# sahngmin/AdaptSegNet

Measured on AMD Instinct MI355X. Metric: adversarial-train images/sec at 1024×512, DeeplabMulti+D, 1/2/4/8 MI355X, higher is better.
Workload: dtype f32; 1 GPU; c2: DeeplabMulti single-level Vanilla, batch/GPU 4, source 1024x512, target 1024x512; global_batch=4, parallelism=dp1, conv_math=f32x3, x3h_mode=3, g16_wide=1, overlap_domains=True, overlap_d=False, target_first=False, d_reuse=True

## Files before the change

adaptsegnet_amd/_lib.py:

```python
from __future__ import annotations

import ctypes
import os
import re
import threading

_HERE = os.path.dirname(os.path.abspath(__file__))
LIB_PATH = os.environ.get("ADAPTSEG_LIBRARY") or os.path.join(_HERE, "lib", "libadaptseg.so")
HEADER_PATH = os.path.join(os.path.dirname(_HERE), "include", "adaptseg.h")

ADAPTSEG_OK = 0
EPI_LEAKY = 1
EPI_ACCUMULATE = 2
EPI_LEAKY_GRAD = 4
EPI_RESIDUAL = 8
EPI_RELU = 16
EPI_RELU_GRAD = 32
CONV_FWD, CONV_BWD_DATA, CONV_BWD_WEIGHT = 0, 1, 2
MATH_F32, MATH_BF16, MATH_BF16_WIDE, MATH_F32X3, MATH_F32X3_PRESPLIT = 0, 1, 2, 3, 4


class AdaptSegLibraryError(RuntimeError):
    pass


class ConvDesc(ctypes.Structure):
    _fields_ = [
        ("n", ctypes.c_int), ("c", ctypes.c_int), ("h", ctypes.c_int), ("w", ctypes.c_int),
        ("in_stride", ctypes.c_int64 * 4),
        ("k", ctypes.c_int), ("oh", ctypes.c_int), ("ow", ctypes.c_int),
        ("kh", ctypes.c_int), ("kw", ctypes.c_int),
        ("stride", ctypes.c_int), ("nseg", ctypes.c_int),
        ("pad", ctypes.c_int * 4), ("dil", ctypes.c_int * 4),
    ]


class OperandBN(ctypes.Structure):
    _fields_ = [("mean", ctypes.c_void_p), ("invstd", ctypes.c_void_p),
                ("weight", ctypes.c_void_p), ("bias", ctypes.c_void_p)]


class BnSumDesc(ctypes.Structure):
    _fields_ = [
        ("x", ctypes.c_void_p), ("x_bf16", ctypes.c_void_p),
        ("mean", ctypes.c_void_p), ("invstd", ctypes.c_void_p),
        ("weight", ctypes.c_void_p), ("bias", ctypes.c_void_p),
        ("bits", ctypes.c_void_p), ("mask", ctypes.c_int),
        ("partial", ctypes.c_void_p), ("partial_bytes", ctypes.c_size_t),
    ]


FUSE_MAX_MAPS = 8
FUSE_PROB, FUSE_LOGIT = 0, 1


class FuseDesc(ctypes.Structure):
    _fields_ = [
        ("n", ctypes.c_int), ("c", ctypes.c_int), ("oh", ctypes.c_int), ("ow", ctypes.c_int),
        ("nmaps", ctypes.c_int), ("mode", ctypes.c_int),
        ("h", ctypes.c_int * FUSE_MAX_MAPS), ("w", ctypes.c_int * FUSE_MAX_MAPS),
        ("mirror", ctypes.c_int * FUSE_MAX_MAPS),
        ("x", ctypes.c_void_p * FUSE_MAX_MAPS),
    ]


_P = ctypes.c_void_p
_I = ctypes.c_int
_L = ctypes.c_int64
_F = ctypes.c_float
_SZ = ctypes.c_size_t
_PP = ctypes.POINTER(ctypes.c_void_p)
_DESC = ctypes.POINTER(ConvDesc)

_SIGS = {
    "adaptseg_last_error": [],
    "adaptseg_version": [],
    "adaptseg_conv2d_workspace_size": [_DESC, _I, ctypes.POINTER(_SZ)],
    "adaptseg_conv2d_kernel_id": [_DESC, _I, ctypes.POINTER(_I), ctypes.POINTER(_I)],
    "adaptseg_conv2d_kernel_id_x": [_DESC, _I, _I, ctypes.POINTER(_I), ctypes.POINTER(_I)],
    "adaptseg_conv2d_copy_operand_only": [_DESC, _I, ctypes.POINTER(_I)],
    "adaptseg_conv2d_operand_bn_ok": [_DESC, _I, ctypes.POINTER(_I)],
    "adaptseg_conv2d_fwd_bnstats_abn": [_DESC, _P, ctypes.POINTER(OperandBN), _PP, _P, _P, _P, _SZ,
                                        ctypes.POINTER(ctypes.c_int), _P, _SZ, _P],
    "adaptseg_conv2d_bwd_weight_abn": [_DESC, _P, _P, ctypes.POINTER(OperandBN), _PP, _I, _P, _SZ, _P],
    "adaptseg_bn_fwd_train_tiles_stats": [_L, _I, _P, _I, _P, _P, _F, _F, _P, _P, _P],
    "adaptseg_conv2d_fwd": [_DESC, _P, _PP, _PP, _P, _P, _I, _P, _SZ, _P],
    "adaptseg_conv2d_bwd_data": [_DESC, _P, _PP, _P, _P, _P, _I, _P, _SZ, _P],
    "adaptseg_conv2d_bwd_weight": [_DESC, _P, _P, _PP, _PP, _I, _P, _SZ, _P],
    "adaptseg_conv2d_wpack_size": [_DESC, _I, ctypes.POINTER(_SZ)],
    "adaptseg_conv2d_wpack": [_DESC, _I, _PP, _P, _SZ, _P],
    "adaptseg_conv2d_fwd_x": [_DESC, _P, _P, _PP, _P, _PP, _P, _P, _P, _I, _P, _SZ, _P],
    "adaptseg_conv2d_fwd_bnstats_x": [_DESC, _P, _P, _PP, _P, _P, _P, _P, _SZ, ctypes.POINTER(ctypes.c_int), _P,
                                      _SZ, _P],
    "adaptseg_conv2d_bwd_data_x": [_DESC, _P, _P, _PP, _P, _P, _P, _P, _P, _I, _P, _SZ, _P],
    "adaptseg_conv2d_bwd_data_xg": [_DESC, _P, _P, _PP, _P, _P, _P, _P, _P, _P, _P, _I, _P, _SZ, _P],
    "adaptseg_conv2d_bwd_weight_x": [_DESC, _P, _P, _P, _P, _PP, _PP, _I, _P, _SZ, _P],
    "adaptseg_conv2d_bnsum_tiles": [_DESC, _I, ctypes.POINTER(_I)],
    "adaptseg_timing_reserve": [_L],
    "adaptseg_conv2d_bwd_data_bnsum": [_DESC, _P, _P, _PP, _P, _P, _P, _P, _P, _P, _I, ctypes.POINTER(BnSumDesc),
                                       ctypes.POINTER(_I), _P, _SZ, _P],
    "adaptseg_bn_bwd_sums": [_L, _I, _P, _P, _P, _P, _P, _P, _P, _P, _P, _P, _P, _P, _P, _P, _P, _I, _P, _I, _P, _SZ,
                             _P],
    "adaptseg_bn_fwd_train_x": [_L, _I, _P, _P, _P, _P, _P, _P, _F, _F, _P, _P, _P, _P, _P, _P, _I, _P, _SZ, _P],
    "adaptseg_bn_fwd_train_tiles_x": [_L, _I, _P, _I, _P, _P, _P, _P, _P, _P, _F, _F, _P, _P, _P, _P, _P, _P, _I,
                                      _P],
    "adaptseg_bn_fwd_infer_x": [_L, _I, _P, _P, _P, _P, _P, _P, _F, _P, _P, _P, _P, _I, _P],
    "adaptseg_bn_fwd_train_xm": [_L, _I, _P, _P, _P, _P, _P, _P, _F, _F, _P, _P, _P, _P, _P, _P, _P, _I, _P, _SZ,
                                 _P],
    "adaptseg_bn_fwd_train_tiles_xm": [_L, _I, _P, _I, _P, _P, _P, _P, _P, _P, _F, _F, _P, _P, _P, _P, _P, _P, _P,
                                       _I, _P],
    "adaptseg_bn_fwd_infer_xm": [_L, _I, _P, _P, _P, _P, _P, _P, _F, _P, _P, _P, _P, _P, _I, _P],
    "adaptseg_bn_bwd_x": [_L, _I, _P, _P, _P, _P, _P, _P, _P, _P, _P, _P, _P, _P, _I, _I, _P, _SZ, _P],
    "adaptseg_bn_bwd_xg": [_L, _I, _P, _P, _P, _P, _P, _P, _P, _P, _P, _P, _P, _P, _P, _P, _P, _I, _I, _P, _SZ, _P],
    "adaptseg_bn_workspace_size": [_L, _I, ctypes.POINTER(_SZ)],
    "adaptseg_bn_fwd_train": [_L, _I, _P, _P, _P, _P, _P, _F, _F, _P, _P, _P, _P, _I, _P, _SZ, _P],
    "adaptseg_upsample_argmax": [_I, _I, _I, _I, _I, _I, _P, _P, _P],
    "adaptseg_fuse_argmax": [ctypes.POINTER(FuseDesc), _P, _P, _P],
    "adaptseg_confusion_hist": [_L, _P, _P, _P, _I, _P, _P],
    "adaptseg_conf_hist": [_L, _P, _P, _I, _I, _P, _P],
    "adaptseg_pseudo_thresholds": [_P, _I, _I, ctypes.c_double, _F, _P, _P],
    "adaptseg_pseudo_label": [_L, _P, _P, _P, _I, _I, _P, _P, _P],
    "adaptseg_bn_fwd_train_tiles": [_L, _I, _P, _I, _P, _P, _P, _P, _P, _F, _F, _P, _P, _P, _P, _I, _P],
    "adaptseg_conv2d_bnstats_size": [_DESC, ctypes.POINTER(ctypes.c_size_t)],
    "adaptseg_conv2d_bnstats_tiles": [_DESC, ctypes.POINTER(_I)],
    "adaptseg_conv2d_bnstats_tiles_x": [_DESC, _I, ctypes.POINTER(_I)],
    "adaptseg_conv2d_fwd_bnstats": [_DESC, _P, _PP, _P, _P, _SZ, ctypes.POINTER(ctypes.c_int), _P, _SZ, _P],
    "adaptseg_bn_fwd_infer": [_L, _I, _P, _P, _P, _P, _P, _F, _P, _P, _I, _P],
    "adaptseg_bn_bwd": [_L, _I, _P, _P, _P, _P, _P, _P, _P, _P, _P, _I, _I, _P, _SZ, _P],
    "adaptseg_maxpool2d_fwd": [_I, _I, _I, _I, _I, _I, _I, _I, _I, _P, _P, _P, _P],
    "adaptseg_maxpool2d_bwd": [_I, _I, _I, _I, _I, _I, _I, _I, _I, _P, _P, _P, _P],
    "adaptseg_maxpool2d_fwd_x": [_I, _I, _I, _I, _I, _I, _I, _I, _I, _P, _P, _P, _P, _P],
    "adaptseg_maxpool2d_bwd_x": [_I, _I, _I, _I, _I, _I, _I, _I, _I, _P, _P, _P, _P, _P],
    "adaptseg_upsample_workspace_size": [_I, _I, _I, _I, _I, _I, ctypes.POINTER(_SZ)],
    "adaptseg_upsample_bilinear_fwd": [_I, _I, _I, _I, _I, _I, _P, _P, _P],
    "adaptseg_upsample_bilinear_bwd": [_I, _I, _I, _I, _I, _I, _P, _P, _I, _P, _SZ, _P],
    "adaptseg_softmax_fwd": [_L, _I, _P, _P, _P],
    "adaptseg_softmax_bwd": [_L, _I, _P, _P, _P, _I, _P],
    "adaptseg_ce_workspace_size": [_L, ctypes.POINTER(_SZ)],
    "adaptseg_softmax_ce_fwd": [_L, _I, _P, _P, _I, _P, _P, _P, _SZ, _P],
    "adaptseg_softmax_ce_bwd": [_L, _I, _P, _P, _I, _P, _P, _P, _P, _I, _P],
    "adaptseg_adv_workspace_size": [_L, ctypes.POINTER(_SZ)],
    "adaptseg_adv_loss_fwd": [_L, _P, _F, _I, _P, _P, _SZ, _P],
    "adaptseg_adv_loss_bwd": [_L, _P, _F, _I, _P, _P, _I, _P],
    "adaptseg_sgd_step": [_L, _P, _P, _P, _F, _F, _F, _F, _I, _I, _P],
    "adaptseg_adam_step": [_L, _P, _P, _P, _P, _F, _F, _F, _F, _I, _F, _P],
    "adaptseg_zero": [_P, _SZ, _P],
    "adaptseg_to_nhwc": [_I, _I, _I, _I, ctypes.POINTER(_L), _P, _P, _P],
    "adaptseg_to_nhwc_pad": [_I, _I, _I, _I, ctypes.POINTER(_L), _P, _I, _P, _I, _P],
    "adaptseg_axpy": [_L, _F, _P, _P, _I, _P],
    "adaptseg_add_i64": [_P, _L, _L, _P],
    "adaptseg_preprocess_workspace_size": [_I, _I, _I, _I, _I, ctypes.POINTER(_SZ)],
    "adaptseg_gta5_preprocess": [_I, _I, _I, _I, _I, _P, _F, _F, _F, _P, _P, _P, _P, _P, _SZ, _P],
    "adaptseg_preprocess_augment_workspace_size": [_I, _I, _I, _I, _I, ctypes.POINTER(ctypes.c_int32),
                                                   ctypes.POINTER(_SZ)],
    "adaptseg_gta5_preprocess_augment": [_I, _I, _I, _I, _I, _P, _F, _F, _F, _P, _P, _P, _P,
                                         ctypes.POINTER(ctypes.c_int32), _I, _P, _SZ, _P],
    "adaptseg_bn_bwd_affine": [_L, _I, _P, _P, _P, _P, _P, _P, _P, _P, _P, _I, _P, _P, _P, _SZ, _P],
    "adaptseg_up2_relu_cat_fwd": [_I, _I, _I, _I, _I, _P, _P, _P, _P],
    "adaptseg_up2_relu_cat_bwd": [_I, _I, _I, _I, _I, _P, _P, _P, _P, _P, _P],
    "adaptseg_grid_warp_fwd": [_I, _I, _I, _I, _I, _P, _P, _P, _P, _P, _P],
    "adaptseg_grid_warp_bwd_workspace_size": [_I, _I, _I, _I, ctypes.POINTER(_SZ)],
    "adaptseg_grid_warp_bwd": [_I, _I, _I, _I, _I, _P, _P, _P, _P, _P, _P, _P, _P, _P, _SZ, _P],
    "adaptseg_conv_set_math": [_I],
    "adaptseg_conv_get_math": [ctypes.POINTER(_I)],
    "adaptseg_conv_set_option": [_I, _I],
    "adaptseg_conv_get_option": [_I, ctypes.POINTER(_I)],
    "adaptseg_splitk_flush": [_P],
    "adaptseg_splitk_pending": [_P, ctypes.POINTER(_I)],
    "adaptseg_stream_create_cu_mask": [_I, _I, ctypes.POINTER(_P)],
    "adaptseg_stream_destroy": [_P],
    "adaptseg_timing_enable": [_I, _I],
    "adaptseg_timing_enable_mem": [_I],
    "adaptseg_timing_read_id": [_I, ctypes.POINTER(ctypes.c_double), ctypes.POINTER(ctypes.c_double),
                                ctypes.POINTER(_L)],
    "adaptseg_timing_read": [ctypes.POINTER(ctypes.c_double), ctypes.POINTER(ctypes.c_double),
                             ctypes.POINTER(_L)],
    "adaptseg_timing_enable_stream": [_I],
    "adaptseg_timing_read_id_stream": [_I, ctypes.POINTER(ctypes.c_double), ctypes.POINTER(_L)],
}
_RESTYPES = {"adaptseg_last_error": ctypes.c_char_p, "adaptseg_version": ctypes.c_char_p}

_lib = None
_lock = threading.Lock()


def header_symbols(path: str = HEADER_PATH) -> list[str]:
    text = open(path).read()
    text = re.sub(r"/\*.*?\*/", "", text, flags=re.S)
    return sorted(set(re.findall(r"\b(adaptseg_[a-z0-9_]+)\s*\(", text)))


def lib():
    global _lib
    if _lib is not None:
        return _lib
    with _lock:
        if _lib is not None:
            return _lib
        if not os.path.exists(LIB_PATH):
            raise AdaptSegLibraryError(
                f"{LIB_PATH} not found: build it with `make -C adaptsegnet_amd/csrc` "
                "(the HIP path has no CPU fallback)")
        try:
            L = ctypes.CDLL(LIB_PATH)
        except OSError as e:
            raise AdaptSegLibraryError(f"failed to load {LIB_PATH}: {e}") from e
        for name, argtypes in _SIGS.items():
            fn = getattr(L, name)
            fn.argtypes = argtypes
            fn.restype = _RESTYPES.get(name, ctypes.c_int)
        _lib = L
        return L


def check(status: int, what: str) -> None:
    if status != ADAPTSEG_OK:
        msg = lib().adaptseg_last_error().decode(errors="replace")
        raise RuntimeError(f"{what} failed (status {status}): {msg}")


def ptr_array(ptrs) -> "ctypes.Array":
    arr = (ctypes.c_void_p * 4)()
    for i, p in enumerate(ptrs):
        arr[i] = p
    return arr
```

adaptsegnet_amd/csrc/conv_igemm.hip:

```cpp
#include <atomic>
#include "conv_kernels.hpp"
#include "conv_thin.hpp"
#include <cstdlib>
#include <mutex>
#include <unordered_map>
#include <vector>

namespace adaptseg {

__global__ void splitk_reduce_kernel(const ConvParams p, const float *slab, int mode) {
  const size_t total = (size_t)p.M * p.N;
  for (size_t idx = blockIdx.x * (size_t)blockDim.x + threadIdx.x; idx < total;
       idx += (size_t)gridDim.x * blockDim.x) {
    float v = 0.f;
    for (int s = 0; s < p.splits; ++s) v += slab[(size_t)s * total + idx];
    int row = (int)(idx / p.N);
    int col = (int)(idx - (size_t)row * p.N);
    if (mode == MODE_WGRAD) {
      int seg = (int)fdiv((uint32_t)col, p.fd_nseg_k);
      int cc = col - seg * p.kseg;
      float *dst = seg == 0 ? p.dw[0] : seg == 1 ? p.dw[1] : seg == 2 ? p.dw[2] : p.dw[3];
      float *o = dst + (size_t)row * p.kseg + cc;
      *o = (p.flags & ADAPTSEG_EPI_ACCUMULATE) ? *o + v : v;
    } else {
// ... 775 lines not shown
static bool terms_in_epilogue(const Plan &pl, const uint16_t *yb, int64_t n) {
  return yb && is_x3(pl.family) && pl.p.N % 4 == 0 && 3 * n < (1ll << 31) && !(reinterpret_cast<uintptr_t>(yb) & 7);
}

static int out_copy(const float *y, uint16_t *yb, int64_t n, int C, hipStream_t s) {
  if (!yb || n == 0) return ADAPTSEG_OK;
  AS_CHECK_ARG(y, "conv: an operand copy needs the fp32 output on this path");
  const unsigned blocks = (unsigned)std::min<int64_t>(ceil_div(n, 256), 8192);
  if (copies_are_terms() && C % 4 == 0 && n / 4 < (1ll << 31) / 3 && aligned16(y) &&
      !(reinterpret_cast<uintptr_t>(yb) & 7))
    x3_out_copy4_kernel<<<(unsigned)std::min<int64_t>(ceil_div(n / 4, 256), 16384), 256, 0, s>>>(
        reinterpret_cast<const float4 *>(y), reinterpret_cast<uint2 *>(yb), (uint32_t)(n / 4), C / 4,
        make_fastdiv(C / 4));
  else if (copies_are_terms())
    x3_out_copy_kernel<<<blocks, 256, 0, s>>>(y, reinterpret_cast<__bf16 *>(yb), n, C);
  else
    bf16_out_copy_kernel<<<blocks, 256, 0, s>>>(y, reinterpret_cast<__bf16 *>(yb), n);
  AS_CHECK_LAUNCH("out_copy");
  return ADAPTSEG_OK;
}

bool use_thin(const adaptseg_conv_desc *d, int op) { return thin_eligible(d, op); }

static bool copy_only(const Plan &pl, const adaptseg_conv_desc *d, int op) {
  if (use_thin(d, op)) return false;
  if (tapgemm_eligible(d)) return tapgemm_copy_only(d, op);
  if (is_x3(pl.family)) return pl.terms_ok;
  return pl.family == Family::Bf16Dma || (pl.family == Family::Bf16 && op == ADAPTSEG_CONV_FWD);
}

static size_t plan_wpack_bytes(const Plan &pl) {
  if (pl.mode == MODE_WGRAD) return 0;
  if (is_x3(pl.family)) return x3_wpack_bytes(pl);
  if (is_bf16(pl.family)) return bf16_wpack_bytes(pl);
  return 0;
}

static int attach_wpack(Plan &pl, const void *w_pack) {
  pl.wpack_ext = nullptr;
  if (!w_pack || plan_wpack_bytes(pl) == 0) return ADAPTSEG_OK;
  AS_CHECK_ARG((reinterpret_cast<uintptr_t>(w_pack) & 15) == 0, "conv: weight pack must be 16-byte aligned");
  pl.wpack_ext = w_pack;
  return ADAPTSEG_OK;
}

static void finish_plan(Plan &pl, bool a_aligned, bool b_aligned, const void *act, const void *act2 = nullptr) {
  const bool two = pl.mode == MODE_WGRAD;
  const bool have = act && aligned16(act) && (!two || (act2 && aligned16(act2)));
  finish_plan(pl, Operands{a_aligned, b_aligned, have});
  pl.act_ext = have ? act : nullptr;
  pl.act_ext2 = have && two ? act2 : nullptr;
}

static int query_plan(const adaptseg_conv_desc *d, int op, const Operands &ops, Plan &pl) {
  const int st = make_plan(d, op, pl);
  if (st == ADAPTSEG_OK) finish_plan(pl, ops);
  return st;
}

}

using namespace adaptseg;

extern "C" {

int adaptseg_conv2d_workspace_size(const adaptseg_conv_desc *d, int op, size_t *bytes) {
  AS_CHECK_ARG(bytes, "null bytes");
  Plan base, pl;
  int st = make_plan(d, op, base);
  if (st) return st;
  size_t b = 0;
  for (const Operands &ops : {Operands{}, Operands{false, false, false}, Operands{true, true, true}}) {
    pl = base;
    finish_plan(pl, ops);
    b = std::max(b, pl.slab_bytes);
  }
  if (tapgemm_eligible(d)) b = std::max(b, tapgemm_workspace(d, op));
  if (use_thin(d, op)) b = std::max(b, thin_workspace(d, op));
  if (op == ADAPTSEG_CONV_BWD_WEIGHT) {
    int per, splits;
    bias_grad_split(d->n * d->oh * d->ow, d->k, &per, &splits);
    b = std::max(b, (size_t)splits * d->k * sizeof(float));
  }
  *bytes = b;
  return ADAPTSEG_OK;
}

int adaptseg_conv2d_kernel_id(const adaptseg_conv_desc *d, int op, int *kernel_id, int *splits) {
  AS_CHECK_ARG(kernel_id && splits, "conv2d_kernel_id: null");
  return adaptseg_conv2d_kernel_id_x(d, op, 0, kernel_id, splits);
}

int adaptseg_conv2d_kernel_id_x(const adaptseg_conv_desc *d, int op, int with_copies, int *kernel_id, int *splits) {
  AS_CHECK_ARG(kernel_id && splits, "conv2d_kernel_id_x: null");
  Plan pl;
  int st = query_plan(d, op, Operands{true, true, with_copies != 0}, pl);
  if (st) return st;
  if (use_thin(d, op)) {
    *kernel_id = thin_kernel_id(op);
    *splits = 1;
    return ADAPTSEG_OK;
  }
  if (tapgemm_eligible(d)) return tapgemm_kernel_id(d, op, kernel_id, splits);
  *kernel_id = ::adaptseg::kernel_id(pl, op);
  *splits = pl.p.splits;
  return ADAPTSEG_OK;
}

static bool abn_plan_ok(const Plan &pl, const adaptseg_conv_desc *d, int op) {
  if (d->c > kAbnMaxC || d->c % 4 || d->nseg != 1 || use_thin(d, op) || tapgemm_eligible(d)) return false;
  return (op == ADAPTSEG_CONV_FWD && pl.family == Family::X3Rows) ||
         (op == ADAPTSEG_CONV_BWD_WEIGHT && pl.family == Family::X3);
}

int adaptseg_conv2d_operand_bn_ok(const adaptseg_conv_desc *d, int op, int *ok) {
  AS_CHECK_ARG(ok, "conv2d_operand_bn_ok: null");
  *ok = 0;
  Plan pl;
  int st = query_plan(d, op, Operands{}, pl);
  if (st) return st;
  if (op != ADAPTSEG_CONV_FWD && op != ADAPTSEG_CONV_BWD_WEIGHT) return ADAPTSEG_OK;
  *ok = abn_plan_ok(pl, d, op) ? 1 : 0;
  return ADAPTSEG_OK;
}

static void set_abn(ConvParams &p, const adaptseg_operand_bn *abn) {
  p.abn_m = abn->mean;
  p.abn_is = abn->invstd;
  p.abn_w = abn->weight;
  p.abn_b = abn->bias;
}

int adaptseg_conv2d_copy_operand_only(const adaptseg_conv_desc *d, int op, int *only) {
  AS_CHECK_ARG(only, "conv2d_copy_operand_only: null");
  *only = 0;
  Plan pl;
  int st = make_plan(d, op, pl);
  if (st) return st;
  *only = copy_only(pl, d, op) ? 1 : 0;
  return ADAPTSEG_OK;
}

int adaptseg_conv2d_wpack_size(const adaptseg_conv_desc *d, int op, size_t *bytes) {
  AS_CHECK_ARG(bytes, "conv2d_wpack_size: null");
  *bytes = 0;
  Plan pl;
  int st = make_plan(d, op, pl);
  if (st) return st;
  if (use_thin(d, op) || tapgemm_eligible(d)) return ADAPTSEG_OK;
  *bytes = plan_wpack_bytes(pl);
  return ADAPTSEG_OK;
}

int adaptseg_conv2d_wpack(const adaptseg_conv_desc *d, int op, const float *const *w, void *pack, size_t bytes,
                          adaptseg_stream_t stream) {
  Plan pl;
  int st = make_plan(d, op, pl);
  if (st) return st;
  AS_CHECK_ARG(w && pack, "conv2d_wpack: null pointer");
  AS_CHECK_ARG((reinterpret_cast<uintptr_t>(pack) & 15) == 0, "conv2d_wpack: pack must be 16-byte aligned");
  const size_t need = (use_thin(d, op) || tapgemm_eligible(d)) ? 0 : plan_wpack_bytes(pl);
  AS_CHECK_ARG(need > 0, "conv2d_wpack: this product reads no weight pack (size 0)");
  AS_CHECK_ARG(bytes >= need, "conv2d_wpack: %zu bytes < %zu", bytes, need);
  for (int s = 0; s < d->nseg; ++s) {
    AS_CHECK_ARG(w[s], "conv2d_wpack: null weight %d", s);
    AS_CHECK_ARG(aligned16(w[s]), "conv2d_wpack: weight %d must be 16-byte aligned", s);
    pl.p.wt[s] = w[s];
  }
  const hipError_t e = is_x3(pl.family) ? prep_x3_wpack(pl, pack, as_stream(stream)) : prep_bf16_wpack(pl, pack, as_stream(stream));
  if (e != hipSuccess) {
    set_error("conv2d_wpack: %s", hipGetErrorString(e));
    return ADAPTSEG_ERR_HIP;
  }
  return ADAPTSEG_OK;
}

int adaptseg_conv2d_fwd(const adaptseg_conv_desc *d, const float *x, const float *const *w,
                        const float *const *bias, const float *res, float *y, int flags, void *ws,
                        size_t ws_bytes, adaptseg_stream_t stream) {
  return adaptseg_conv2d_fwd_x(d, x, nullptr, w, nullptr, bias, res, y, nullptr, flags, ws, ws_bytes, stream);
}

struct FwdStats {
  float *stats;
  size_t stats_bytes;
  int *ntiles;
  const adaptseg_operand_bn *abn;
};

static int fwd_impl(const adaptseg_conv_desc *d, const float *x, const uint16_t *x_bf16, const float *const *w,
                    const void *w_pack, const float *const *bias, const float *res, float *y, uint16_t *y_bf16,
                    int flags, void *ws, size_t ws_bytes, adaptseg_stream_t stream, const FwdStats *bn) {
  const char *who = bn ? "conv fwd_bnstats" : "conv fwd";
  if (bn) {
    AS_CHECK_ARG(bn->ntiles && bn->stats, "conv fwd_bnstats: null stats / ntiles");
    *bn->ntiles = 0;
  }
  Plan pl;
  int st = make_plan(d, ADAPTSEG_CONV_FWD, pl);
  if (st) return st;
  const bool thin = !bn && use_thin(d, ADAPTSEG_CONV_FWD);
  AS_CHECK_ARG((x || x_bf16) && w && (y || y_bf16), "%s: null pointer", who);
  AS_CHECK_ARG(y || !(thin || tapgemm_eligible(d)), "%s: this product needs the fp32 output%s", who,
               bn ? "" : " (thin / tap-GEMM path)");
  AS_CHECK_ARG(y || !(flags & ADAPTSEG_EPI_ACCUMULATE), "conv fwd: ACCUMULATE needs the fp32 output");
  AS_CHECK_ARG(x || copy_only(pl, d, ADAPTSEG_CONV_FWD),
               "%s: this product needs the fp32 input (no bf16-operand kernel for it)", who);
  AS_CHECK_ARG(!(flags & kEpiActGrad), "conv fwd: *_GRAD flags not valid");
  AS_CHECK_ARG(!((flags & ADAPTSEG_EPI_LEAKY) && (flags & ADAPTSEG_EPI_RELU)), "conv fwd: LEAKY and RELU");
  AS_CHECK_ARG(!(flags & ADAPTSEG_EPI_RESIDUAL) || res, "conv fwd: residual flag without res");
  for (int s = 0; s < d->nseg; ++s) AS_CHECK_ARG(w[s], "%s: null weight %d", who, s);
  AS_CHECK_ARG(!bn || !bn->abn || !tapgemm_eligible(d), "conv fwd_bnstats_abn: no operand-BN kernel for this product");
  if (bn && tapgemm_eligible(d))
    return fwd_impl(d, x, x_bf16, w, nullptr, nullptr, nullptr, y, y_bf16, 0, ws, ws_bytes, stream, nullptr);
  const int64_t ny = (int64_t)d->n * d->oh * d->ow * d->k;
  if (thin && thin_fwd(d, x, w[0], bias ? bias[0] : nullptr, res, y, flags, as_stream(stream)) == ADAPTSEG_OK)
    return out_copy(y, y_bf16, ny, d->k, as_stream(stream));
  if (tapgemm_eligible(d) && aligned16(x) && segs_aligned(w, d->nseg)) {
    st = tapgemm_fwd(d, x, x_bf16, w, bias, res, y, flags, ws, ws_bytes, as_stream(stream));
    return st ? st : out_copy(y, y_bf16, ny, d->k, as_stream(stream));
  }
  ConvParams &p = pl.p;
  p.x = x;
  for (int s = 0; s < d->nseg; ++s) {
    p.wt[s] = w[s];
    p.bias[s] = bias ? bias[s] : nullptr;
  }
  finish_plan(pl, aligned16(x), segs_aligned(w, d->nseg), x_bf16);
  AS_CHECK_ARG(x || (copy_only(pl, d, ADAPTSEG_CONV_FWD) && pl.act_ext),
               "%s: x is NULL but the plan (after the alignment checks) needs the fp32 input", who);
  if (bn && bn->abn) {
    AS_CHECK_ARG(abn_plan_ok(pl, d, ADAPTSEG_CONV_FWD),
                 "conv fwd_bnstats_abn: no operand-BN kernel for this product (adaptseg_conv2d_operand_bn_ok)");
    set_abn(p, bn->abn);
  }
  const bool terms = copies_are_terms();
  AS_CHECK_ARG(y || !terms, "%s: under the F32X3 maths the output is fp32%s", who,
               bn ? "" : " (y_bf16 is its term images)");
  const bool fused = terms && terms_in_epilogue(pl, y_bf16, ny);
  p.out = y;
  p.outb = (terms && !fused) ? nullptr : reinterpret_cast<__bf16 *>(y_bf16);
  p.outb_terms = fused ? 1 : 0;
  p.res = res;
  p.flags = flags;
  if (bn && pl.family != Family::Generic && p.splits == 1) {
    const int nt = (int)ceil_div(p.M, pl.tile.bm);
    if ((size_t)(nt + 2 * (int64_t)p.N * nt) * sizeof(float) <= bn->stats_bytes) {
      p.stats = bn->stats;
      p.stats_ntiles = nt;
      *bn->ntiles = nt;
    }
  }
  st = attach_wpack(pl, w_pack);
  if (st) return st;
  st = run_plan(pl, MODE_FWD, ws, ws_bytes, as_stream(stream));
  return (st || !terms || fused) ? st : out_copy(y, y_bf16, ny, d->k, as_stream(stream));
}

int adaptseg_conv2d_fwd_x(const adaptseg_conv_desc *d, const float *x, const uint16_t *x_bf16,
                          const float *const *w, const void *w_pack, const float *const *bias, const float *res,
                          float *y, uint16_t *y_bf16, int flags, void *ws, size_t ws_bytes,
                          adaptseg_stream_t stream) {
  return fwd_impl(d, x, x_bf16, w, w_pack, bias, res, y, y_bf16, flags, ws, ws_bytes, stream, nullptr);
}

int adaptseg_conv2d_bnstats_size(const adaptseg_conv_desc *d, size_t *bytes) {
  AS_CHECK_ARG(bytes, "conv2d_bnstats_size: null");
  int st = validate(d);
  if (st) return st;
  const int64_t m = (int64_t)d->n * d->oh * d->ow;
  const int64_t nt = ceil_div(m, 128);
  *bytes = (size_t)(nt + 2 * (int64_t)d->k * nt) * sizeof(float);
  return ADAPTSEG_OK;
}

int adaptseg_conv2d_bnstats_tiles(const adaptseg_conv_desc *d, int *ntiles) {
  return adaptseg_conv2d_bnstats_tiles_x(d, 0, ntiles);
}

int adaptseg_conv2d_bnstats_tiles_x(const adaptseg_conv_desc *d, int with_copy, int *ntiles) {
  AS_CHECK_ARG(ntiles, "conv2d_bnstats_tiles: null");
  *ntiles = 0;
  Plan pl;
  int st = query_plan(d, ADAPTSEG_CONV_FWD, Operands{true, true, with_copy != 0}, pl);
  if (st) return st;
  if (tapgemm_eligible(d)) return ADAPTSEG_OK;
  if (pl.family != Family::Generic && pl.p.splits == 1) *ntiles = (int)ceil_div(pl.p.M, pl.tile.bm);
  return ADAPTSEG_OK;
}

int adaptseg_conv2d_fwd_bnstats(const adaptseg_conv_desc *d, const float *x, const float *const *w, float *y,
                                float *stats, size_t stats_bytes, int *ntiles, void *ws, size_t ws_bytes,
                                adaptseg_stream_t stream) {
  return adaptseg_conv2d_fwd_bnstats_x(d, x, nullptr, w, nullptr, y, nullptr, stats, stats_bytes, ntiles, ws, ws_bytes,
                                       stream);
}

int adaptseg_conv2d_fwd_bnstats_x(const adaptseg_conv_desc *d, const float *x, const uint16_t *x_bf16,
                                  const float *const *w, const void *w_pack, float *y, uint16_t *y_bf16,
                                  float *stats, size_t stats_bytes, int *ntiles, void *ws, size_t ws_bytes,
                                  adaptseg_stream_t stream) {
  const FwdStats bn{stats, stats_bytes, ntiles, nullptr};
  return fwd_impl(d, x, x_bf16, w, w_pack, nullptr, nullptr, y, y_bf16, 0, ws, ws_bytes, stream, &bn);
}

int adaptseg_conv2d_fwd_bnstats_abn(const adaptseg_conv_desc *d, const float *x_pre, const adaptseg_operand_bn *abn,
                                    const float *const *w, const void *w_pack, float *y, float *stats,
                                    size_t stats_bytes, int *ntiles, void *ws, size_t ws_bytes,
                                    adaptseg_stream_t stream) {
  AS_CHECK_ARG(abn && abn->mean && abn->invstd && x_pre, "conv fwd_bnstats_abn: null operand BN / input");
  const FwdStats bn{stats, stats_bytes, ntiles, abn};
  return fwd_impl(d, x_pre, nullptr, w, w_pack, nullptr, nullptr, y, nullptr, 0, ws, ws_bytes, stream, &bn);
}

int adaptseg_conv2d_bwd_data(const adaptseg_conv_desc *d, const float *dy, const float *const *w,
                             const float *res, const float *aux, float *dx, int flags, void *ws,
                             size_t ws_bytes, adaptseg_stream_t stream) {
  return adaptseg_conv2d_bwd_data_x(d, dy, nullptr, w, nullptr, res, aux, dx, nullptr, flags, ws, ws_bytes, stream);
}

int adaptseg_conv2d_bwd_data_x(const adaptseg_conv_desc *d, const float *dy, const uint16_t *dy_bf16,
                               const float *const *w, const void *w_pack, const float *res, const float *aux,
                               float *dx, uint16_t *dx_bf16, int flags, void *ws, size_t ws_bytes,
                               adaptseg_stream_t stream) {
// ... 410 lines not shown
```

adaptsegnet_amd/csrc/conv_kernels.hpp:

```cpp
#pragma once
#include "common.hpp"
#include <algorithm>
#include <cstring>

namespace adaptseg {


typedef float floatx16 __attribute__((ext_vector_type(16)));

enum { MODE_FWD = 0, MODE_DGRAD = 1, MODE_WGRAD = 2 };
constexpr int kMaxTaps = 64;
constexpr int BK = 16;
constexpr int kX3BK = 16;
constexpr int kX3rBK = 32;
constexpr int x3_bn(int mode) { return 128; }
constexpr int x3_threads(int mode) { return 512; }

struct ConvParams {
  int M, N, K;
  int n, c, h, w;
  int sxn, sxc, sxh, sxw;
  int k, oh, ow;
  int stride;
  int ntaps, taps_per_seg, nseg;
  int kseg;
  int ktiles_per_split, splits;
  FastDiv fd_c, fd_k, fd_ow, fd_oh, fd_ohw, fd_hw, fd_w, fd_nseg_k;
  const float *x;
  const float *dy;
  const float *wt[4];
  float *out;
  float *dw[4];
  const float *bias[4];
  const float *res;
  const __bf16 *resb;
  const uint32_t *resbits;
  const float *aux;
  int flags;
  int kw_, kh_;
  int pad_[4], dil_[4];
  FastDiv fd_taps, fd_kw;
  __bf16 *outb;
  int outb_terms;
  float *stats;
  int stats_ntiles;
  float *bs_part;
  const float *bs_x;
  const __bf16 *bs_xb;
  const float *bs_mean, *bs_is, *bs_w, *bs_b;
  const uint32_t *bs_bits;
  int bs_mask, bs_ntiles;
  short tap_dy[kMaxTaps], tap_dx[kMaxTaps];
  const float *abn_m, *abn_is, *abn_w, *abn_b;
};
constexpr int kAbnMaxC = 512;

__device__ __forceinline__ float epi_prev(const ConvParams &p, size_t idx) {
  return p.out ? p.out[idx] : (float)p.outb[idx];
}
__device__ __forceinline__ void epi_outb(const ConvParams &p, size_t row, int col, float v) {
  if (p.outb_terms) {
    uint32_t h, m, l;
    split3_2(v, 0.f, h, m, l);
    __bf16 *o = p.outb + row * 3 * p.N + col;
    o[0] = __builtin_bit_cast(__bf16, (uint16_t)h);
    o[p.N] = __builtin_bit_cast(__bf16, (uint16_t)m);
    o[2 * p.N] = __builtin_bit_cast(__bf16, (uint16_t)l);
  } else {
    p.outb[row * p.N + col] = (__bf16)v;
  }
}
__device__ __forceinline__ float epi_res(const ConvParams &p, size_t idx) {
  const float r = p.resb ? (float)p.resb[idx] : p.res[idx];
  return (!p.resbits || ((p.resbits[idx >> 5] >> (idx & 31)) & 1u)) ? r : 0.f;
}


__device__ __forceinline__ float4 ld4(const float *p) { return *reinterpret_cast<const float4 *>(p); }

struct RowInfo {
  int base;
  int y0, x0;
  bool ok;
};

__device__ __forceinline__ RowInfo fwd_row_info(const ConvParams &p, int m) {
  RowInfo r;
  r.ok = m < p.M;
  int mm = r.ok ? m : 0;
  uint32_t t = fdiv((uint32_t)mm, p.fd_ow);
  int ow = mm - (int)t * p.ow;
  uint32_t b = fdiv(t, p.fd_oh);
  int oh = (int)t - (int)b * p.oh;
  r.base = (int)b * p.sxn;
  r.y0 = oh * p.stride;
  r.x0 = ow * p.stride;
  return r;
}

__device__ __forceinline__ float fwd_a_elem(const ConvParams &p, const short *tdy, const short *tdx,
                                            const RowInfo &r, int k) {
  if (!r.ok || k >= p.K) return 0.f;
  int tap = (int)fdiv((uint32_t)k, p.fd_c);
  int ci = k - tap * p.c;
  int ih = r.y0 + tdy[tap], iw = r.x0 + tdx[tap];
  if ((unsigned)ih >= (unsigned)p.h || (unsigned)iw >= (unsigned)p.w) return 0.f;
  return p.x[r.base + ih * p.sxh + iw * p.sxw + ci * p.sxc];
}

template <bool VEC>
__device__ __forceinline__ float4 fwd_a_load(const ConvParams &p, const short *tdy, const short *tdx,
                                             const RowInfo &r, int k) {
  if constexpr (VEC) {
    if (!r.ok || k >= p.K) return make_float4(0.f, 0.f, 0.f, 0.f);
    int tap = (int)fdiv((uint32_t)k, p.fd_c);
    int ci = k - tap * p.c;
    int ih = r.y0 + tdy[tap], iw = r.x0 + tdx[tap];
    if ((unsigned)ih >= (unsigned)p.h || (unsigned)iw >= (unsigned)p.w)
      return make_float4(0.f, 0.f, 0.f, 0.f);
    return ld4(p.x + r.base + ih * p.sxh + iw * p.sxw + ci);
  } else {
    return make_float4(fwd_a_elem(p, tdy, tdx, r, k), fwd_a_elem(p, tdy, tdx, r, k + 1),
                       fwd_a_elem(p, tdy, tdx, r, k + 2), fwd_a_elem(p, tdy, tdx, r, k + 3));
  }
}

__device__ __forceinline__ const float *seg_ptr(const ConvParams &p, int seg) {
  return seg == 0 ? p.wt[0] : seg == 1 ? p.wt[1] : seg == 2 ? p.wt[2] : p.wt[3];
}

__device__ __forceinline__ float fwd_b_elem(const ConvParams &p, int n, int k) {
  if (n >= p.N || k >= p.K) return 0.f;
  int seg = (int)fdiv((uint32_t)k, p.fd_nseg_k);
  int kk = k - seg * p.kseg;
  return seg_ptr(p, seg)[n * p.kseg + kk];
}

template <bool VEC>
__device__ __forceinline__ float4 fwd_b_load(const ConvParams &p, int n, int k) {
  if constexpr (VEC) {
    if (n >= p.N || k >= p.K) return make_float4(0.f, 0.f, 0.f, 0.f);
    int seg = (int)fdiv((uint32_t)k, p.fd_nseg_k);
    int kk = k - seg * p.kseg;
    return ld4(seg_ptr(p, seg) + n * p.kseg + kk);
  } else {
    return make_float4(fwd_b_elem(p, n, k), fwd_b_elem(p, n, k + 1), fwd_b_elem(p, n, k + 2),
                       fwd_b_elem(p, n, k + 3));
  }
}

__device__ __forceinline__ RowInfo dgrad_row_info(const ConvParams &p, int m) {
  RowInfo r;
  r.ok = m < p.M;
  int mm = r.ok ? m : 0;
  uint32_t t = fdiv((uint32_t)mm, p.fd_w);
  int iw = mm - (int)t * p.w;
  uint32_t b = fdiv(t, p.fd_hw);
  int ih = (int)t - (int)b * p.h;
  r.base = (int)b;
  r.y0 = ih;
  r.x0 = iw;
  return r;
}

__device__ __forceinline__ bool dgrad_src(const ConvParams &p, int v, int d, int lim, int &o) {
  int num = v - d;
  if (p.stride == 1) {
    o = num;
  } else {
    if (num < 0 || (num % p.stride) != 0) return false;
    o = num / p.stride;
  }
  return (unsigned)o < (unsigned)lim;
}

__device__ __forceinline__ float dgrad_a_elem(const ConvParams &p, const short *tdy, const short *tdx,
                                              const RowInfo &r, int k) {
  if (!r.ok || k >= p.K) return 0.f;
  int tap = (int)fdiv((uint32_t)k, p.fd_k);
  int co = k - tap * p.k;
  int oh, ow;
  if (!dgrad_src(p, r.y0, tdy[tap], p.oh, oh) || !dgrad_src(p, r.x0, tdx[tap], p.ow, ow)) return 0.f;
  return p.dy[((r.base * p.oh + oh) * p.ow + ow) * p.k + co];
}

template <bool VEC>
__device__ __forceinline__ float4 dgrad_a_load(const ConvParams &p, const short *tdy, const short *tdx,
                                               const RowInfo &r, int k) {
  if constexpr (VEC) {
    if (!r.ok || k >= p.K) return make_float4(0.f, 0.f, 0.f, 0.f);
    int tap = (int)fdiv((uint32_t)k, p.fd_k);
    int co = k - tap * p.k;
    int oh, ow;
    if (!dgrad_src(p, r.y0, tdy[tap], p.oh, oh) || !dgrad_src(p, r.x0, tdx[tap], p.ow, ow))
      return make_float4(0.f, 0.f, 0.f, 0.f);
    return ld4(p.dy + ((r.base * p.oh + oh) * p.ow + ow) * p.k + co);
  } else {
    return make_float4(dgrad_a_elem(p, tdy, tdx, r, k), dgrad_a_elem(p, tdy, tdx, r, k + 1),
                       dgrad_a_elem(p, tdy, tdx, r, k + 2), dgrad_a_elem(p, tdy, tdx, r, k + 3));
  }
}

__device__ __forceinline__ const float *dgrad_b_row(const ConvParams &p, int k) {
  int tap = (int)fdiv((uint32_t)k, p.fd_k);
  int co = k - tap * p.k;
  int seg = tap / p.taps_per_seg;
  int t = tap - seg * p.taps_per_seg;
  return seg_ptr(p, seg) + (co * p.taps_per_seg + t) * p.c;
}
// ... 1251 lines not shown
        d[2 * SA] = v.z;
        d[3 * SA] = v.w;
      } else {
        *reinterpret_cast<float4 *>(As + a_k[i] * SA + a_col[i]) = v;
      }
    }
#pragma unroll
    for (int i = 0; i < NQB; ++i) {
      const float4 v = mask4(mb[i], rb[i]);
      if constexpr (B_KC) {
        float *d = Bs + b_k[i] * SB + b_col[i];
        d[0] = v.x;
        d[SB] = v.y;
        d[2 * SB] = v.z;
        d[3 * SB] = v.w;
      } else {
        *reinterpret_cast<float4 *>(Bs + b_k[i] * SB + b_col[i]) = v;
      }
    }
  };

  const int lane = tid & 63, wave = tid >> 6;
  const int wm = wave / WAVES_N, wn = wave - wm * WAVES_N;
  const int l32 = lane & 31, hh = lane >> 5;

  floatx16 acc[TM][TN];
#pragma unroll
  for (int i = 0; i < TM; ++i)
#pragma unroll
    for (int j = 0; j < TN; ++j)
#pragma unroll
      for (int r = 0; r < 16; ++r) acc[i][j][r] = 0.f;

  if (kt0 < kt1) {
    load_tile(kt0);
    store_tile(0);
    __syncthreads();
    int cur = 0;
    for (int kt = kt0; kt < kt1; ++kt) {
      const bool more = kt + 1 < kt1;
      if (more) load_tile(kt + 1);
      const float *As = lds + cur * STAGE + wm * WTM + l32;
      const float *Bs = lds + cur * STAGE + BK * SA + wn * WTN + l32;
      float a[2][TM], b[2][TN];
#pragma unroll
      for (int i = 0; i < TM; ++i) a[0][i] = As[hh * SA + i * 32];
#pragma unroll
      for (int j = 0; j < TN; ++j) b[0][j] = Bs[hh * SB + j * 32];
      __builtin_amdgcn_s_setprio(1);
#pragma unroll
      for (int kk = 0; kk < BK; kk += 2) {
        const int cb = (kk >> 1) & 1;
        if (kk + 2 < BK) {
#pragma unroll
          for (int i = 0; i < TM; ++i) a[cb ^ 1][i] = As[(kk + 2 + hh) * SA + i * 32];
#pragma unroll
          for (int j = 0; j < TN; ++j) b[cb ^ 1][j] = Bs[(kk + 2 + hh) * SB + j * 32];
        }
        __builtin_amdgcn_sched_barrier(0);
#pragma unroll
        for (int i = 0; i < TM; ++i)
#pragma unroll
          for (int j = 0; j < TN; ++j)
            acc[i][j] = __builtin_amdgcn_mfma_f32_32x32x2f32(a[cb][i], b[cb][j], acc[i][j], 0, 0, 0);
      }
      __builtin_amdgcn_s_setprio(0);
      if (more) store_tile(cur ^ 1);
      __syncthreads();
      cur ^= 1;
    }
  }

  igemm_epilogue<MODE, BM, BN, WAVES_M, WAVES_N, S2>(p, acc, bm, bn, tm, tn, split, M, Hc, Wc, py, px, lds);
}


enum class Family {
  Generic,
  Fast,
  Bf16,
  Bf16Dma,
  X3,
  X3Terms,
  X3Rows,
};
inline bool is_x3(Family f) { return f == Family::X3 || f == Family::X3Terms || f == Family::X3Rows; }
inline bool is_bf16(Family f) { return f == Family::Bf16 || f == Family::Bf16Dma; }

struct Tile {
  int bm, bn, bk, threads;
};

struct Plan {
  ConvParams p;
  Family family;
  Tile tile;
  int cfg;
  bool va, vb;
  bool s2;
  bool ae, be;
  bool terms_ok;
  bool act_caller;
  const void *act_ext;
  const void *act_ext2;
  const void *wpack_ext;
  int mode;
  int tiles;
  size_t slab_bytes;
  double flops;
};

struct Operands {
  bool a_aligned = true, b_aligned = true;
  bool copies = false;
};

static const int kCfgBM[9] = {128, 256, 32, 64, 256, 64, 128, 256, 128};
static const int kCfgBN[9] = {128, 32, 256, 256, 64, 64, 128, 128, 128};
static const int kCfgThreads[9] = {256, 256, 256, 256, 256, 256, 256, 512, 256};
static int fast_bk(int cfg) { return (cfg == 4 || cfg == 6 || cfg == 8) ? 16 : 32; }


double conv_flops(const adaptseg_conv_desc *d);
int make_plan(const adaptseg_conv_desc *d, int op, Plan &pl);
void finish_plan(Plan &pl, const Operands &ops);
void set_splits(Plan &pl);
int kernel_id(const Plan &pl, int mode);
int run_plan(Plan &pl, int mode, void *ws, size_t ws_bytes, hipStream_t s, bool defer = false);

bool tapgemm_eligible(const adaptseg_conv_desc *d);
bool tapgemm_copy_only(const adaptseg_conv_desc *d, int op);
size_t tapgemm_workspace(const adaptseg_conv_desc *d, int op);
int tapgemm_kernel_id(const adaptseg_conv_desc *d, int op, int *kid, int *splits);
int tapgemm_fwd(const adaptseg_conv_desc *d, const float *x, const uint16_t *x_bf16, const float *const *w,
                const float *const *bias, const float *res, float *y, int flags, void *ws, size_t ws_bytes,
                hipStream_t s);
int tapgemm_bwd_data(const adaptseg_conv_desc *d, const float *dy, const float *const *w, const float *res,
                     const float *aux, float *dx, int flags, void *ws, size_t ws_bytes, hipStream_t s);
int tapgemm_bwd_weight(const adaptseg_conv_desc *d, const float *dy, const float *x, const uint16_t *x_bf16,
                       float *const *dw, int flags, void *ws, size_t ws_bytes, hipStream_t s);

hipError_t launch_fwd(const Plan &pl, hipStream_t s);
int conv_math();
size_t bf16_wpack_bytes(const Plan &pl);
size_t bf16_pre_bytes(const Plan &pl);
hipError_t prep_bf16(Plan &pl, void *ws, hipStream_t s);
hipError_t prep_bf16_wpack(const Plan &pl, void *pack, hipStream_t s);
hipError_t launch_bf16(const Plan &pl, void *ws, hipStream_t s);
size_t x3_wpack_bytes(const Plan &pl);
size_t x3_pre_bytes(const Plan &pl);
hipError_t prep_x3(const Plan &pl, void *wpack, hipStream_t s);
hipError_t prep_x3_wpack(const Plan &pl, void *pack, hipStream_t s);
hipError_t launch_x3(const Plan &pl, void *wpack, hipStream_t s);
hipError_t launch_dgrad(const Plan &pl, hipStream_t s);
hipError_t launch_wgrad(const Plan &pl, hipStream_t s);

}
```

adaptsegnet_amd/csrc/conv_launch_bf16.hip:

```cpp
#include "conv_bf16.hpp"
#include "conv_bf16g.hpp"

namespace adaptseg {

__global__ void conv_wpack_fwd_kernel(const ConvParams p, __bf16 *out) {
  const int ktot = p.nseg * p.kseg;
  const int64_t n = (int64_t)p.k * ktot;
  for (int64_t i = (int64_t)blockIdx.x * blockDim.x + threadIdx.x; i < n; i += (int64_t)gridDim.x * blockDim.x) {
    const int co = (int)(i / ktot), kk = (int)(i - (int64_t)co * ktot);
    const int seg = kk / p.kseg, tk = kk - seg * p.kseg;
    out[i] = (__bf16)seg_ptr(p, seg)[(size_t)co * p.kseg + tk];
  }
}

__global__ void __launch_bounds__(256) conv_wpack_dgrad_kernel(const ConvParams p, __bf16 *out) {
  __shared__ float tile[64][65];
  const int ci0 = blockIdx.x * 64, co0 = blockIdx.y * 64, tap = blockIdx.z;
  const int seg = tap / p.taps_per_seg, t = tap - seg * p.taps_per_seg;
  const float *w = seg_ptr(p, seg);
  const int tx = threadIdx.x & 63, ty = threadIdx.x >> 6;
  for (int r = ty; r < 64; r += 4) {
    const int co = co0 + r, ci = ci0 + tx;
    tile[r][tx] = (co < p.k && ci < p.c) ? w[((size_t)co * p.taps_per_seg + t) * p.c + ci] : 0.f;
  }
  __syncthreads();
  const size_t ktot = (size_t)p.ntaps * p.k;
  for (int r = ty; r < 64; r += 4) {
    const int ci = ci0 + r, co = co0 + tx;
    if (ci < p.c && co < p.k) out[(size_t)ci * ktot + (size_t)tap * p.k + co] = (__bf16)tile[tx][r];
  }
}

__global__ void __launch_bounds__(256) conv_wpack_fwd_v_kernel(const ConvParams p, uint4 *__restrict__ out,
                                                               uint32_t cpr, uint32_t total) {
  for (uint32_t i = blockIdx.x * 256u + threadIdx.x; i < total; i += gridDim.x * 256u) {
    const uint32_t co = i / cpr, k0 = (i - co * cpr) * 8;
    int seg = 0;
    uint32_t tk = k0;
    while (tk >= (uint32_t)p.kseg) { tk -= p.kseg; ++seg; }
    const float *src = seg_ptr(p, seg) + (size_t)co * p.kseg + tk;
    const uint2 lo = cvt4_bf16(ld4(src)), hi = cvt4_bf16(ld4(src + 4));
    out[i] = make_uint4(lo.x, lo.y, hi.x, hi.y);
  }
}

__global__ void __launch_bounds__(256) conv_wpack_dgrad_v_kernel(const ConvParams p, __bf16 *out) {
  __shared__ float tile[64][65];
  const int ci0 = blockIdx.x * 64, co0 = blockIdx.y * 64, tap = blockIdx.z;
  const int seg = tap / p.taps_per_seg, t = tap - seg * p.taps_per_seg;
  const float *w = seg_ptr(p, seg);
  const int f = threadIdx.x & 15, r0 = threadIdx.x >> 4;
#pragma unroll
  for (int j = 0; j < 4; ++j) {
    const int r = r0 + 16 * j, co = co0 + r, ci = ci0 + 4 * f;
    float4 v = make_float4(0.f, 0.f, 0.f, 0.f);
    if (co < p.k && ci < p.c) v = ld4(w + ((size_t)co * p.taps_per_seg + t) * p.c + ci);
    tile[r][4 * f] = v.x; tile[r][4 * f + 1] = v.y; tile[r][4 * f + 2] = v.z; tile[r][4 * f + 3] = v.w;
  }
  __syncthreads();
  const size_t ktot = (size_t)p.ntaps * p.k;
  const int c = threadIdx.x & 7, co = co0 + 8 * c;
#pragma unroll
  for (int j = 0; j < 2; ++j) {
    const int rl = (threadIdx.x >> 3) + 32 * j, ci = ci0 + rl;
    if (ci >= p.c || co >= p.k) continue;
    const float *col = &tile[8 * c][rl];
    const uint2 lo = cvt4_bf16(make_float4(col[0], col[65], col[130], col[195]));
    const uint2 hi = cvt4_bf16(make_float4(col[260], col[325], col[390], col[455]));
    *reinterpret_cast<uint4 *>(out + (size_t)ci * ktot + (size_t)tap * p.k + co) = make_uint4(lo.x, lo.y, hi.x, hi.y);
  }
}

__global__ void bf16_copy_kernel(const float *__restrict__ x, int n, int h, int w, int c8, int sxn, int sxh,
                                 int sxw, uint4 *__restrict__ out) {
  const int64_t total = (int64_t)n * h * w * c8;
  for (int64_t i = (int64_t)blockIdx.x * blockDim.x + threadIdx.x; i < total; i += (int64_t)gridDim.x * blockDim.x) {
    const int cq = (int)(i % c8);
    const int64_t pix = i / c8;
    const int xx = (int)(pix % w);
    const int64_t t = pix / w;
    const int yy = (int)(t % h), b = (int)(t / h);
    const float *src = x + (int64_t)b * sxn + (int64_t)yy * sxh + (int64_t)xx * sxw + 8 * cq;
    const uint2 lo = cvt4_bf16(ld4(src)), hi = cvt4_bf16(ld4(src + 4));
    out[i] = make_uint4(lo.x, lo.y, hi.x, hi.y);
  }
}

static size_t g16_act_elems(const Plan &pl) {
  const ConvParams &p = pl.p;
  if (pl.family != Family::Bf16Dma) return 0;
  return pl.mode == MODE_FWD ? (size_t)p.n * p.h * p.w * p.c : (size_t)p.n * p.oh * p.ow * p.k;
}
static size_t g16_act2_elems(const Plan &pl) {
  const ConvParams &p = pl.p;
  return pl.family == Family::Bf16Dma && pl.mode == MODE_WGRAD ? (size_t)p.n * p.h * p.w * p.c : 0;
}
static size_t al256(size_t b) { return (b + 255) / 256 * 256; }

size_t bf16_pre_bytes(const Plan &pl) {
  return al256(bf16_wpack_bytes(pl)) + al256(g16_act_elems(pl) * sizeof(__bf16)) +
         al256(g16_act2_elems(pl) * sizeof(__bf16));
}

size_t bf16_wpack_bytes(const Plan &pl) {
  const ConvParams &p = pl.p;
  if (pl.mode == MODE_FWD) return (size_t)p.k * p.nseg * p.kseg * sizeof(__bf16);
  if (pl.mode == MODE_DGRAD) return (size_t)p.c * p.ntaps * p.k * sizeof(__bf16);
  return 0;
}

hipError_t prep_bf16_wpack(const Plan &pl, void *pack, hipStream_t s) {
  const ConvParams &p = pl.p;
  __bf16 *wb = reinterpret_cast<__bf16 *>(pack);
  bool wal = true;
  for (int g = 0; g < p.nseg; ++g) wal = wal && (reinterpret_cast<uintptr_t>(p.wt[g]) & 15) == 0;
  if (pl.mode == MODE_FWD) {
    const int64_t n = (int64_t)p.k * p.nseg * p.kseg;
    if (wal && p.kseg % 8 == 0 && n / 8 < (int64_t)1 << 31) {
      const uint32_t total = (uint32_t)(n / 8);
      conv_wpack_fwd_v_kernel<<<(unsigned)std::min<int64_t>(ceil_div(total, 256), 4096), 256, 0, s>>>(
          p, reinterpret_cast<uint4 *>(wb), (uint32_t)(p.nseg * p.kseg / 8), total);
    } else {
      conv_wpack_fwd_kernel<<<(unsigned)std::min<int64_t>(ceil_div(n, 256), 4096), 256, 0, s>>>(p, wb);
    }
  } else if (pl.mode == MODE_DGRAD) {
    dim3 g((unsigned)ceil_div(p.c, 64), (unsigned)ceil_div(p.k, 64), (unsigned)p.ntaps);
    if (wal && p.c % 4 == 0 && p.k % 8 == 0) conv_wpack_dgrad_v_kernel<<<g, 256, 0, s>>>(p, wb);
    else conv_wpack_dgrad_kernel<<<g, 256, 0, s>>>(p, wb);
  }
  return hipGetLastError();
}

hipError_t prep_bf16(Plan &pl, void *wpack, hipStream_t s) {
  const ConvParams &p = pl.p;
  if (!pl.wpack_ext) {
    const hipError_t e = prep_bf16_wpack(pl, wpack, s);
    if (e != hipSuccess) return e;
  }
  if (pl.family == Family::Bf16Dma) {
    char *base = reinterpret_cast<char *>(wpack) + al256(bf16_wpack_bytes(pl));
    uint4 *act = reinterpret_cast<uint4 *>(base);
    const int64_t n8 = (int64_t)g16_act_elems(pl) / 8;
    const unsigned blocks = (unsigned)std::min<int64_t>(ceil_div(n8, 256), 8192);
    if (!pl.act_ext) {
      if (pl.mode == MODE_FWD)
        bf16_copy_kernel<<<blocks, 256, 0, s>>>(p.x, p.n, p.h, p.w, p.c / 8, p.sxn, p.sxh, p.sxw, act);
      else
        bf16_copy_kernel<<<blocks, 256, 0, s>>>(p.dy, p.n, p.oh, p.ow, p.k / 8, p.oh * p.ow * p.k, p.ow * p.k,
                                                p.k, act);
    }
    if (pl.mode == MODE_WGRAD && !pl.act_ext2) {
      uint4 *act2 = reinterpret_cast<uint4 *>(base + al256(g16_act_elems(pl) * sizeof(__bf16)));
      const int64_t m8 = (int64_t)g16_act2_elems(pl) / 8;
      bf16_copy_kernel<<<(unsigned)std::min<int64_t>(ceil_div(m8, 256), 8192), 256, 0, s>>>(
          p.x, p.n, p.h, p.w, p.c / 8, p.sxn, p.sxh, p.sxw, act2);
    }
  }
  return hipGetLastError();
}

hipError_t launch_bf16(const Plan &pl, void *wpack, hipStream_t s) {
  const ConvParams &p = pl.p;
  const __bf16 *wb = reinterpret_cast<const __bf16 *>(pl.wpack_ext ? pl.wpack_ext : wpack);
  const Tile &t = pl.tile;
  const bool bn256 = t.bn == 256;
  dim3 grid(pl.tiles, p.splits, pl.s2 ? 4 : 1), block(t.threads);
  if (pl.family == Family::Bf16Dma) {
    const char *base = reinterpret_cast<const char *>(wpack) + al256(bf16_wpack_bytes(pl));
    const __bf16 *act = reinterpret_cast<const __bf16 *>(pl.act_ext ? pl.act_ext : base);
    if (pl.s2) {
      if (bn256) launch_k(igemm_bf16g_kernel<MODE_DGRAD, 128, 256, 32, true>, grid, block, s, p, act, wb);
      else launch_k(igemm_bf16g_kernel<MODE_DGRAD, 256, 128, 32, true>, grid, block, s, p, act, wb);
    } else if (pl.mode == MODE_WGRAD) {
      const __bf16 *act2 = reinterpret_cast<const __bf16 *>(
          pl.act_ext2 ? pl.act_ext2 : base + al256(g16_act_elems(pl) * sizeof(__bf16)));
      if (bn256) launch_k(igemm_bf16g_wgrad_kernel<256, 256, 2>, grid, block, s, p, act, act2);
      else if (t.bm == 256) launch_k(igemm_bf16g_wgrad_kernel<256>, grid, block, s, p, act, act2);
      else launch_k(igemm_bf16g_wgrad_kernel<128>, grid, block, s, p, act, act2);
    } else {
#define G16_LAUNCH(MODE_, BK_)                                                                     \
  do {                                                                                             \
    if (t.bm == 256 && bn256)                                                                      \
      launch_k(igemm_bf16g_kernel<MODE_, 256, 256, 64, false, 2>, grid, block, s, p, act, wb);     \
    else if (bn256) launch_k(igemm_bf16g_kernel<MODE_, 128, 256, BK_>, grid, block, s, p, act, wb); \
    else launch_k(igemm_bf16g_kernel<MODE_, 256, 128, BK_>, grid, block, s, p, act, wb);           \
  } while (0)
      if (pl.mode == MODE_FWD && t.bk == 64) G16_LAUNCH(MODE_FWD, 64);
      else if (pl.mode == MODE_FWD) G16_LAUNCH(MODE_FWD, 32);
      else if (t.bk == 64) G16_LAUNCH(MODE_DGRAD, 64);
      else G16_LAUNCH(MODE_DGRAD, 32);
#undef G16_LAUNCH
    }
    return hipGetLastError();
  }
  const __bf16 *act = pl.mode == MODE_FWD ? reinterpret_cast<const __bf16 *>(pl.act_ext) : nullptr;
  if (pl.mode == MODE_FWD && act) {
    if (bn256) launch_k(igemm_bf16_kernel<MODE_FWD, false, 256, true>, grid, block, s, p, wb, act);
    else launch_k(igemm_bf16_kernel<MODE_FWD, false, 128, true>, grid, block, s, p, wb, act);
  } else if (pl.mode == MODE_FWD) {
    if (bn256) launch_k(igemm_bf16_kernel<MODE_FWD, false, 256>, grid, block, s, p, wb, act);
    else launch_k(igemm_bf16_kernel<MODE_FWD, false, 128>, grid, block, s, p, wb, act);
  } else if (pl.mode == MODE_DGRAD && pl.s2) {
    if (bn256) launch_k(igemm_bf16_kernel<MODE_DGRAD, true, 256>, grid, block, s, p, wb, act);
    else launch_k(igemm_bf16_kernel<MODE_DGRAD, true, 128>, grid, block, s, p, wb, act);
  } else if (pl.mode == MODE_DGRAD) {
    if (bn256) launch_k(igemm_bf16_kernel<MODE_DGRAD, false, 256>, grid, block, s, p, wb, act);
    else launch_k(igemm_bf16_kernel<MODE_DGRAD, false, 128>, grid, block, s, p, wb, act);
  } else {
    launch_k(igemm_bf16_kernel<MODE_WGRAD, false, 128>, grid, block, s, p, wb, act);
  }
  return hipGetLastError();
}

}
```

adaptsegnet_amd/csrc/conv_launch_x3.hip:

```cpp
#include "conv_x3r.hpp"

namespace adaptseg {

static void x3_pack_dims(const Plan &pl, int &rows_pad, int &ktot) {
  const ConvParams &p = pl.p;
  rows_pad = ktot = 0;
  if (pl.mode == MODE_FWD) {
    rows_pad = (int)ceil_div(p.k, x3_bn(MODE_FWD)) * x3_bn(MODE_FWD);
    ktot = p.nseg * p.kseg;
  } else if (pl.mode == MODE_DGRAD) {
    rows_pad = (int)ceil_div(p.c, x3_bn(MODE_DGRAD)) * x3_bn(MODE_DGRAD);
    ktot = p.ntaps * p.k;
  }
}

size_t x3_wpack_bytes(const Plan &pl) {
  int rows_pad, ktot;
  x3_pack_dims(pl, rows_pad, ktot);
  return 3 * (size_t)rows_pad * ktot * sizeof(__bf16);
}

static size_t x3_act_elems(const Plan &pl) {
  const ConvParams &p = pl.p;
  if (pl.family != Family::X3Terms) return 0;
  return pl.mode == MODE_FWD ? (size_t)p.n * p.h * p.w * p.c : (size_t)p.n * p.oh * p.ow * p.k;
}
static size_t x3_act2_elems(const Plan &pl) {
  const ConvParams &p = pl.p;
  return pl.family == Family::X3Terms && pl.mode == MODE_WGRAD ? (size_t)p.n * p.h * p.w * p.c : 0;
}
static size_t al256(size_t b) { return (b + 255) / 256 * 256; }

size_t x3_pre_bytes(const Plan &pl) {
  if (pl.act_caller) return al256(x3_wpack_bytes(pl));
  return al256(x3_wpack_bytes(pl)) + al256(3 * x3_act_elems(pl) * sizeof(__bf16)) +
         al256(3 * x3_act2_elems(pl) * sizeof(__bf16));
}

static void split_copy(const float *x, int n, int h, int w, int c, int sxn, int sxh, int sxw, void *out,
                       hipStream_t s) {
  const int64_t n8 = (int64_t)n * h * w * c / 8;
  x3_split_copy_kernel<<<(unsigned)std::min<int64_t>(ceil_div(n8, 256), 8192), 256, 0, s>>>(
      x, n, h, w, c / 8, sxn, sxh, sxw, reinterpret_cast<uint4 *>(out));
}

hipError_t prep_x3_wpack(const Plan &pl, void *pack, hipStream_t s) {
  const ConvParams &p = pl.p;
  int rows_pad, ktot;
  x3_pack_dims(pl, rows_pad, ktot);
  const dim3 pg((unsigned)(rows_pad / x3_bn(pl.mode)), (unsigned)(ktot / kX3BK));
  if (pl.mode == MODE_FWD) conv_wpack_x3v_kernel<MODE_FWD><<<pg, 256, 0, s>>>(p, (char *)pack, ktot);
  else if (pl.mode == MODE_DGRAD) conv_wpack_x3v_kernel<MODE_DGRAD><<<pg, 256, 0, s>>>(p, (char *)pack, ktot);
  return hipGetLastError();
}

hipError_t prep_x3(const Plan &pl, void *wpack, hipStream_t s) {
  const ConvParams &p = pl.p;
  if (!pl.wpack_ext) {
    const hipError_t e = prep_x3_wpack(pl, wpack, s);
    if (e != hipSuccess) return e;
  }
  if (pl.family == Family::X3Terms) {
    char *base = reinterpret_cast<char *>(wpack) + al256(x3_wpack_bytes(pl));
    if (!pl.act_ext) {
      if (pl.mode == MODE_FWD) split_copy(p.x, p.n, p.h, p.w, p.c, p.sxn, p.sxh, p.sxw, base, s);
      else split_copy(p.dy, p.n, p.oh, p.ow, p.k, p.oh * p.ow * p.k, p.ow * p.k, p.k, base, s);
    }
    if (pl.mode == MODE_WGRAD && !pl.act_ext2)
      split_copy(p.x, p.n, p.h, p.w, p.c, p.sxn, p.sxh, p.sxw, base + al256(3 * x3_act_elems(pl) * sizeof(__bf16)),
                 s);
  }
  return hipGetLastError();
}

hipError_t launch_x3(const Plan &pl, void *wpack, hipStream_t s) {
  const ConvParams &p = pl.p;
  const __bf16 *wb = reinterpret_cast<const __bf16 *>(pl.wpack_ext ? pl.wpack_ext : wpack);
  const int mode = pl.mode;
  dim3 grid(pl.tiles, p.splits, pl.s2 ? 4 : 1), block(pl.tile.threads);
  switch (pl.family) {
    case Family::X3Terms: {
      const char *base = reinterpret_cast<const char *>(wpack) + al256(x3_wpack_bytes(pl));
      const __bf16 *act = reinterpret_cast<const __bf16 *>(pl.act_ext ? pl.act_ext : base);
      if (mode == MODE_FWD) launch_k(igemm_x3r_kernel<MODE_FWD, false>, grid, block, s, p, act, wb);
      else if (mode == MODE_DGRAD && pl.s2) launch_k(igemm_x3r_kernel<MODE_DGRAD, true>, grid, block, s, p, act, wb);
      else if (mode == MODE_DGRAD) launch_k(igemm_x3r_kernel<MODE_DGRAD, false>, grid, block, s, p, act, wb);
      else {
        const __bf16 *act2 = reinterpret_cast<const __bf16 *>(
            pl.act_ext2 ? pl.act_ext2 : base + al256(3 * x3_act_elems(pl) * sizeof(__bf16)));
        if (pl.tile.bm == 256) launch_k(igemm_x3r_wgrad_kernel<256>, grid, block, s, p, act, act2);
        else launch_k(igemm_x3r_wgrad_kernel<128>, grid, block, s, p, act, act2);
      }
      break;
    }
    case Family::X3Rows:
      if (mode == MODE_WGRAD) launch_k(igemm_x3hw_kernel<128>, grid, block, s, p);
      else if (mode == MODE_FWD && p.abn_m) launch_k(igemm_x3h_abn_kernel, grid, block, s, p, wb);
      else if (mode == MODE_FWD) launch_k(igemm_x3h_kernel<MODE_FWD, false>, grid, block, s, p, wb);
      else if (pl.s2) launch_k(igemm_x3h_kernel<MODE_DGRAD, true>, grid, block, s, p, wb);
      else launch_k(igemm_x3h_kernel<MODE_DGRAD, false>, grid, block, s, p, wb);
      break;
    case Family::X3:
      if (mode == MODE_FWD) launch_k(igemm_x3_kernel<MODE_FWD, false>, grid, block, s, p, wb);
      else if (mode == MODE_DGRAD && pl.s2) launch_k(igemm_x3_kernel<MODE_DGRAD, true>, grid, block, s, p, wb);
      else if (mode == MODE_DGRAD) launch_k(igemm_x3_kernel<MODE_DGRAD, false>, grid, block, s, p, wb);
      else if (p.abn_m) launch_k(igemm_x3_abn_kernel, grid, block, s, p, wb);
      else launch_k(igemm_x3_kernel<MODE_WGRAD, false>, grid, block, s, p, wb);
      break;
    default: return hipErrorInvalidValue;
  }
  return hipGetLastError();
}

}
```

adaptsegnet_amd/csrc/conv_x3.hpp:

```cpp
#pragma once
#include "conv_bf16.hpp"


namespace adaptseg {

constexpr int kX3Img = 128 * kX3BK * 2;

__device__ __forceinline__ int kc16_off(int r, int ch) { return r * 32 + ((ch ^ ((r >> 3) & 1)) << 4); }

__device__ __forceinline__ bf16x8 kc16_frag(const char *img, int r0, int lane) {
  return as_bf16x8(*reinterpret_cast<const uint4 *>(img + kc16_off(r0 + (lane & 31), lane >> 5)));
}

typedef unsigned int u32x4 __attribute__((ext_vector_type(4)));
static __device__ __attribute__((aligned(16))) float g_x3_zero4[4];

template <int MODE, bool S2, bool ABN>
__device__ __forceinline__ void x3_body(const ConvParams &p, const __bf16 *__restrict__ wb) {
  static_assert(!ABN || MODE == MODE_WGRAD, "operand BN: the weight gradient's x operand");
  constexpr bool MC = MODE == MODE_WGRAD;
  constexpr int BM = 128, BN = 128, BK = kX3BK, NT = x3_threads(MODE);
  constexpr int WAVES_M = 2, WAVES_N = NT / 128;
  constexpr int WTM = BM / WAVES_M, WTN = BN / WAVES_N;
  constexpr int TM = WTM / 32, TN = WTN / 32;
// ... 204 lines not shown
        uint2 h, m, l;
        split3(ra[i], h, m, l);
        *reinterpret_cast<uint2 *>(As + o) = h;
        *reinterpret_cast<uint2 *>(As + IMG + o) = m;
        *reinterpret_cast<uint2 *>(As + 2 * IMG + o) = l;
        split3(rbf[i], h, m, l);
        *reinterpret_cast<uint2 *>(Bs + o) = h;
        *reinterpret_cast<uint2 *>(Bs + IMGB + o) = m;
        *reinterpret_cast<uint2 *>(Bs + 2 * IMGB + o) = l;
      }
    }
  };

  const int lane = tid & 63, wave = tid >> 6;
  const int wm = wave / WAVES_N, wn = wave - wm * WAVES_N;
  uint32_t mca[MC ? TM : 1][2], mcb[MC ? TN : 1][2];
  if constexpr (MC) {
    const int g = lane >> 4, i16 = lane & 15, q = i16 >> 2, pp = i16 & 3;
    const int kb = 8 * (g >> 1);
    auto offs = [&](int c0, uint32_t (&o)[2]) {
      const int ch = ((c0 + 16 * (g & 1)) >> 3) + (pp >> 1);
      o[0] = (uint32_t)(mc_off(kb + q, ch) + 8 * (pp & 1));
      o[1] = (uint32_t)(mc_off(kb + 4 + q, ch) + 8 * (pp & 1));
    };
#pragma unroll
    for (int i = 0; i < TM; ++i) offs(wm * WTM + i * 32, mca[i]);
#pragma unroll
    for (int j = 0; j < TN; ++j) offs(wn * WTN + j * 32, mcb[j]);
  }
  const uint32_t lds_u32 = (uint32_t)(uintptr_t)lds;
  auto mc_read = [&](uint32_t img_base, const uint32_t (&o)[2]) -> bf16x8 {
    const bf16x4 t0 = __builtin_amdgcn_ds_read_tr16_b64_v4bf16((lds_bf16x4 *)(uintptr_t)(img_base + o[0]));
    const bf16x4 t1 = __builtin_amdgcn_ds_read_tr16_b64_v4bf16((lds_bf16x4 *)(uintptr_t)(img_base + o[1]));
    return __builtin_shufflevector(t0, t1, 0, 1, 2, 3, 4, 5, 6, 7);
  };

  floatx16 acc[TM][TN];
#pragma unroll
  for (int i = 0; i < TM; ++i)
#pragma unroll
    for (int j = 0; j < TN; ++j)
#pragma unroll
      for (int r = 0; r < 16; ++r) acc[i][j][r] = 0.f;
  floatx16 accs[TM][TN];
#pragma unroll
  for (int i = 0; i < TM; ++i)
#pragma unroll
    for (int j = 0; j < TN; ++j)
#pragma unroll
      for (int r = 0; r < 16; ++r) accs[i][j][r] = 0.f;

  auto abn_x = [&]() {
    if constexpr (ABN) {
      const float *L = reinterpret_cast<const float *>(lds + 2 * STAGE) + b_off[0];
      const float4 bm4 = *reinterpret_cast<const float4 *>(L);
      const float4 bi4 = *reinterpret_cast<const float4 *>(L + kAbnMaxC);
      const float4 bw4 = *reinterpret_cast<const float4 *>(L + 2 * kAbnMaxC);
      const float4 bb4 = *reinterpret_cast<const float4 *>(L + 3 * kAbnMaxC);
      float4 &xv = rbf[0];
      xv.x = rbv ? bn_relu(xv.x, bm4.x, bi4.x, bw4.x, bb4.x) : 0.f;
      xv.y = rbv ? bn_relu(xv.y, bm4.y, bi4.y, bw4.y, bb4.y) : 0.f;
      xv.z = rbv ? bn_relu(xv.z, bm4.z, bi4.z, bw4.z, bb4.z) : 0.f;
      xv.w = rbv ? bn_relu(xv.w, bm4.w, bi4.w, bw4.w, bb4.w) : 0.f;
    }
  };
  auto compute = [&](auto cur_c) {
    constexpr int cur = decltype(cur_c)::value;
    const char *As = lds + cur * STAGE;
    const char *Bs = As + 3 * IMG;
    abn_x();
    bf16x8 a[3][TM], b[3][TN];
#pragma unroll
    for (int s = 0; s < 3; ++s) {
#pragma unroll
      for (int i = 0; i < TM; ++i) {
        if constexpr (MC) a[s][i] = mc_read(lds_u32 + cur * STAGE + s * IMG, mca[i]);
        else a[s][i] = kc16_frag(As + s * IMG, wm * WTM + i * 32, lane);
      }
#pragma unroll
      for (int j = 0; j < TN; ++j) {
        if constexpr (MC) b[s][j] = mc_read(lds_u32 + cur * STAGE + 3 * IMG + s * IMGB, mcb[j]);
        else b[s][j] = kc16_frag(Bs + s * IMGB, wn * WTN + j * 32, lane);
      }
    }
    constexpr int TA[6] = {0, 0, 1, 0, 1, 2};
    constexpr int TB[6] = {0, 1, 0, 2, 1, 0};
    __builtin_amdgcn_s_setprio(1);
#pragma unroll
    for (int u = 0; u < 6; ++u)
#pragma unroll
      for (int i = 0; i < TM; ++i)
#pragma unroll
        for (int j = 0; j < TN; ++j) {
          if (u == 0) acc[i][j] = __builtin_amdgcn_mfma_f32_32x32x16_bf16(a[0][i], b[0][j], acc[i][j], 0, 0, 0);
          else accs[i][j] = __builtin_amdgcn_mfma_f32_32x32x16_bf16(a[TA[u]][i], b[TB[u]][j], accs[i][j], 0, 0, 0);
        }
    store_tile(std::integral_constant<int, cur ^ 1>{});
#pragma unroll
    for (int q = 0; q < 6 * TM * TN; ++q) {
      __builtin_amdgcn_sched_group_barrier(0x008, 1, 0);
      __builtin_amdgcn_sched_group_barrier(0x002, 3, 0);
      __builtin_amdgcn_sched_group_barrier(0x200, 1, 0);
    }
    __builtin_amdgcn_s_setprio(0);
  };

  if constexpr (ABN) {
    float *L = reinterpret_cast<float *>(lds + 2 * STAGE);
    for (int c = tid; c < p.c; c += NT) {
      L[c] = p.abn_m[c];
      L[kAbnMaxC + c] = p.abn_is[c];
      L[2 * kAbnMaxC + c] = p.abn_w ? p.abn_w[c] : 1.f;
      L[3 * kAbnMaxC + c] = p.abn_b ? p.abn_b[c] : 0.f;
    }
    __syncthreads();
  }
  if (kt0 < kt1) {
    const int klast = kt1 - 1;
    load_tile(kt0);
    abn_x();
    store_tile(std::integral_constant<int, 0>{});
    load_tile(min(kt0 + 1, klast));
    __syncthreads();
    for (int kt = kt0; kt < kt1; kt += 2) {
      compute(std::integral_constant<int, 0>{});
      load_tile(min(kt + 2, klast));
      __syncthreads();
      if (kt + 1 >= kt1) break;
      compute(std::integral_constant<int, 1>{});
      load_tile(min(kt + 3, klast));
      __syncthreads();
    }
  }

#pragma unroll
  for (int i = 0; i < TM; ++i)
#pragma unroll
    for (int j = 0; j < TN; ++j) acc[i][j] += accs[i][j];
  static_assert(sizeof(lds) >= WAVES_M * WAVES_N * 32 * 36 * 4, "LDS for the f32x4 epilogue");
  igemm_epilogue<MODE, BM, BN, WAVES_M, WAVES_N, S2, 2>(p, acc, bm, bn, tm, tn, split, M, Hc, Wc, py, px,
                                                      reinterpret_cast<float *>(lds));
}

template <int MODE, bool S2>
__global__ void __launch_bounds__(x3_threads(MODE), 4) igemm_x3_kernel(const ConvParams p, const __bf16 *__restrict__ wb) {
  x3_body<MODE, S2, false>(p, wb);
}
__global__ void __launch_bounds__(x3_threads(MODE_WGRAD), 4) igemm_x3_abn_kernel(const ConvParams p,
                                                                               const __bf16 *__restrict__ wb) {
  x3_body<MODE_WGRAD, false, true>(p, wb);
}

template <int MODE>
__global__ void __launch_bounds__(256) conv_wpack_x3v_kernel(const ConvParams p, char *out, int ktot) {
  constexpr int TR = x3_bn(MODE), IMGB = TR * kX3BK * 2;
  const int r = threadIdx.x >> 1, ch = threadIdx.x & 1;
  const int n = blockIdx.x * TR + r;
  const int ks = blockIdx.y, k0 = ks * kX3BK + 8 * ch;
  float v[8];
  if constexpr (MODE == MODE_FWD) {
    if (n < p.k) {
      const int seg = k0 / p.kseg;
      const float *src = seg_ptr(p, seg) + (size_t)n * p.kseg + (k0 - seg * p.kseg);
      const float4 a = ld4(src), b = ld4(src + 4);
      v[0] = a.x; v[1] = a.y; v[2] = a.z; v[3] = a.w; v[4] = b.x; v[5] = b.y; v[6] = b.z; v[7] = b.w;
    } else {
#pragma unroll
      for (int j = 0; j < 8; ++j) v[j] = 0.f;
    }
  } else {
    const int tap = k0 / p.k, co = k0 - tap * p.k;
    const int seg = tap / p.taps_per_seg, t = tap - seg * p.taps_per_seg;
    const float *src = seg_ptr(p, seg) + ((size_t)co * p.taps_per_seg + t) * p.c + n;
    const size_t cs = (size_t)p.taps_per_seg * p.c;
#pragma unroll
    for (int j = 0; j < 8; ++j) v[j] = n < p.c ? src[j * cs] : 0.f;
  }
  uint4 h, m, l;
  split3_2(v[0], v[1], h.x, m.x, l.x);
  split3_2(v[2], v[3], h.y, m.y, l.y);
  split3_2(v[4], v[5], h.z, m.z, l.z);
  split3_2(v[6], v[7], h.w, m.w, l.w);
  const int nkt = ktot / kX3BK;
  char *dst = out + ((size_t)blockIdx.x * nkt + ks) * 3 * IMGB + kc16_off(r, ch);
  *reinterpret_cast<uint4 *>(dst) = h;
  *reinterpret_cast<uint4 *>(dst + IMGB) = m;
  *reinterpret_cast<uint4 *>(dst + 2 * IMGB) = l;
}

}
```

adaptsegnet_amd/kernels.py:

```python
from __future__ import annotations

import contextlib
import ctypes
import weakref
from dataclasses import dataclass

import torch

from . import _lib
from . import ops as _ops
from ._lib import (CONV_BWD_DATA, CONV_BWD_WEIGHT, CONV_FWD, EPI_ACCUMULATE, EPI_LEAKY,
                   EPI_LEAKY_GRAD, EPI_RELU, EPI_RELU_GRAD, EPI_RESIDUAL, MATH_BF16, MATH_BF16_WIDE, MATH_F32, MATH_F32X3, MATH_F32X3_PRESPLIT,
                   ConvDesc, check)

__all__ = [
    "ConvGeom", "set_conv_math", "get_conv_math", "MATH_F32", "MATH_BF16", "MATH_BF16_WIDE", "MATH_F32X3", "MATH_F32X3_PRESPLIT", "conv_fwd", "conv_fwd_bnstats", "conv_dgrad", "conv_wgrad", "bn_fwd_train",
    "bn_fwd_train_tiles", "bn_fwd_infer", "bn_bwd",
    "maxpool_fwd", "maxpool_bwd", "upsample_fwd", "upsample_bwd", "softmax_fwd", "softmax_bwd",
    "ce_fwd", "ce_bwd", "adv_fwd", "adv_bwd", "sgd_step", "adam_step", "zero_", "to_nhwc",
    "axpy", "add_i64", "weight_pack_scope", "pack_builds", "pack_count", "clear_weight_packs", "EPI_ACCUMULATE", "EPI_LEAKY", "EPI_LEAKY_GRAD", "EPI_RELU", "EPI_RELU_GRAD", "EPI_RESIDUAL",
]


_OP = _ops.OPS
_p, _stream, _ws_args, workspace = _ops._p, _ops._stream, _ops._ws_args, _ops.workspace


def _require(t: torch.Tensor, what: str):
    if not t.is_cuda:
        raise RuntimeError(f"{what}: expected a CUDA (HIP) tensor, got device {t.device}")
    if t.dtype != torch.float32:
        raise RuntimeError(f"{what}: expected float32, got {t.dtype}")


@dataclass(frozen=True)
class ConvGeom:

    cin: int
    cout: int
    kh: int
    kw: int
    stride: int = 1
    pads: tuple = (0,)
    dils: tuple = (1,)

    @property
    def nseg(self) -> int:
        return len(self.pads)

    def out_hw(self, h: int, w: int):
        p, d = self.pads[0], self.dils[0]
        oh = (h + 2 * p - d * (self.kh - 1) - 1) // self.stride + 1
        ow = (w + 2 * p - d * (self.kw - 1) - 1) // self.stride + 1
        return oh, ow

    def flops(self, n: int, h: int, w: int) -> float:
        oh, ow = self.out_hw(h, w)
        return 2.0 * n * oh * ow * self.cout * self.cin * self.kh * self.kw * self.nseg


def set_conv_math(math: int) -> None:
    _ops.set_math(math)


def set_x3h(mode: int) -> None:
    _ops.set_option(_ops.OPT_X3H, mode)


def get_x3h() -> int:
    return _ops.get_option(_ops.OPT_X3H)


def set_g16_wide(mode) -> None:
    _ops.set_option(_ops.OPT_G16_WIDE, 3 if mode is True else int(mode))


def get_g16_wide() -> int:
    return _ops.get_option(_ops.OPT_G16_WIDE)


def get_conv_math() -> int:
    m = ctypes.c_int(0)
    check(_lib.lib().adaptseg_conv_get_math(ctypes.byref(m)), "conv_get_math")
    return m.value


def _desc(g: ConvGeom, n, h, w, strides):
    return _ops.conv_desc(n, g.cin, h, w, strides, g.cout, g.kh, g.kw, g.stride, g.pads, g.dils)


class _PackCache:

    def __init__(self):
        self.depth = 0
        self.epoch = 0
        self.entries = {}
        self.finalizers = {}
        self.sizes = {}
        self.builds = 0

    def _drop(self, wid):
        self.entries.pop(wid, None)
        self.finalizers.pop(wid, None)

    def track(self, weight):
        wid = id(weight)
        per = self.entries.get(wid)
        if per is None:
            per = self.entries[wid] = {}
            f = self.finalizers.get(wid)
            if f is None or not f.alive:
                self.finalizers[wid] = weakref.finalize(weight, self._drop, wid)
        return per


_PACKS = _PackCache()


@contextlib.contextmanager
def weight_pack_scope():
    _PACKS.depth += 1
    try:
        yield
    finally:
        _PACKS.depth -= 1
        if _PACKS.depth == 0:
            _PACKS.epoch += 1


def pack_builds() -> int:
    return _PACKS.builds


def pack_count() -> int:
    return sum(len(v) for v in list(_PACKS.entries.values()))


def clear_weight_packs() -> None:
    _PACKS.entries.clear()


def _wpack(g, n, h, w, strides, weights, op):
    if _PACKS.depth == 0:
        return None
    if not _aligned16(*weights):
        return None
    math = _ops._CONV_MATH[0]
    skey = (g, op, math, strides[1] == 1)
    size = _PACKS.sizes.get(skey)
    if size is None:
        d = _desc(g, n, h, w, tuple(strides))[0]
        b = ctypes.c_size_t(0)
        check(_lib.lib().adaptseg_conv2d_wpack_size(ctypes.byref(d), op, ctypes.byref(b)), "conv2d_wpack_size")
        size = _PACKS.sizes[skey] = b.value
    if size == 0:
        return None
    per = _PACKS.track(weights[0])
    key = (tuple(t.data_ptr() for t in weights), g, op, math)
    e = per.get(key)
    if e is None or e[0].numel() < size:
        e = per[key] = [torch.empty(size, dtype=torch.uint8, device=weights[0].device), -1]
    if e[1] != _PACKS.epoch:
        _OP.conv2d_wpack(list(weights), e[0], (n, g.cin, h, w), tuple(strides), _wshape(g), g.stride, g.pads,
                         g.dils, op)
        e[1] = _PACKS.epoch
        _PACKS.builds += 1
    return e[0]


def nhwc_strides(n, h, w, c):
    return (h * w * c, 1, w * c, c)


def _wshape(g: ConvGeom):
    return (g.cout, g.cin, g.kh, g.kw)


def conv_fwd(g: ConvGeom, x: torch.Tensor, n: int, h: int, w: int, weights, biases=None,
             strides=None, out=None, res=None, flags: int = 0, xb=None, bf16_out: bool = False,
             bf16_only: bool = False):
    strides = strides or nhwc_strides(n, h, w, g.cin)
    oh, ow = g.out_hw(h, w)
    dev = (x if x is not None else xb).device
    if bf16_only:
        outb = torch.empty((n, oh, ow, g.cout), device=dev, dtype=torch.bfloat16)
        wp = _wpack(g, n, h, w, strides, weights, CONV_FWD)
        _OP.conv2d_fwd(x, xb, list(weights), wp, list(biases) if biases is not None else [], res, None, outb,
                       (n, g.cin, h, w), strides, _wshape(g), g.stride, g.pads, g.dils,
                       flags | (EPI_RESIDUAL if res is not None else 0))
        return outb
    if out is None:
        out = torch.empty((n, oh, ow, g.cout), device=dev, dtype=torch.float32)
    if res is not None:
        flags |= EPI_RESIDUAL
    outb = _bf16_like(out, bf16_out)
    wp = _wpack(g, n, h, w, strides, weights, CONV_FWD)
    _OP.conv2d_fwd(x, xb, list(weights), wp, list(biases) if biases is not None else [], res, out, outb,
                   (n, g.cin, h, w), strides, _wshape(g), g.stride, g.pads, g.dils, flags)
    return (out, outb) if bf16_out else out


def conv_bnstats_tiles(g: ConvGeom, n: int, h: int, w: int, strides, with_copy: bool = False) -> int:
    d = _desc(g, n, h, w, tuple(strides))[0]
    nt = ctypes.c_int(0)
    check(_lib.lib().adaptseg_conv2d_bnstats_tiles_x(ctypes.byref(d), 1 if with_copy else 0, ctypes.byref(nt)),
          "conv2d_bnstats_tiles")
    return nt.value


def conv_fwd_bnstats(g: ConvGeom, x: torch.Tensor, n: int, h: int, w: int, weights, strides=None, xb=None,
                     bf16_only: bool = False):
    strides = tuple(strides or nhwc_strides(n, h, w, g.cin))
    nt = conv_bnstats_tiles(g, n, h, w, strides, with_copy=xb is not None and _aligned16(xb))
    if nt == 0 or not _aligned16(x, *weights):
        return conv_fwd(g, x, n, h, w, weights, strides=strides, xb=xb, bf16_only=bf16_only), None
    oh, ow = g.out_hw(h, w)
    dev = (x if x is not None else xb).device
    shape = (n, oh, ow, g.cout)
    out = None if bf16_only else torch.empty(shape, device=dev, dtype=torch.float32)
    outb = torch.empty(shape, device=dev, dtype=torch.bfloat16) if bf16_only else None
    stats = torch.empty(nt * (1 + 2 * g.cout), device=dev, dtype=torch.float32)
    wp = _wpack(g, n, h, w, strides, weights, CONV_FWD)
    _OP.conv2d_fwd_bnstats(x, xb, list(weights), wp, out, outb, stats, (n, g.cin, h, w), strides, _wshape(g),
                           g.stride, g.pads, g.dils, nt)
    return (outb if bf16_only else out), (stats, nt)


def _aligned16(*ts) -> bool:
    return all(t is None or t.data_ptr() % 16 == 0 for t in ts)


@dataclass
class OperandBN:
    mean: torch.Tensor
    invstd: torch.Tensor
    weight: torch.Tensor | None
    bias: torch.Tensor | None


def operand_bn_ok(g: ConvGeom, n: int, h: int, w: int, op: int) -> bool:
    return _ops.operand_bn_ok((n, g.cin, h, w), nhwc_strides(n, h, w, g.cin), _wshape(g), g.stride, g.pads, g.dils,
                              op)


def conv_fwd_bnstats_abn(g: ConvGeom, x_pre: torch.Tensor, abn: OperandBN, n: int, h: int, w: int, weights):
    strides = nhwc_strides(n, h, w, g.cin)
    nt = conv_bnstats_tiles(g, n, h, w, strides)
    if nt == 0 or not _aligned16(x_pre, *weights):
        raise RuntimeError("conv_fwd_bnstats_abn: no fused-statistics plan for this product / unaligned operand")
    oh, ow = g.out_hw(h, w)
    out = torch.empty((n, oh, ow, g.cout), device=x_pre.device, dtype=torch.float32)
    stats = torch.empty(nt * (1 + 2 * g.cout), device=x_pre.device, dtype=torch.float32)
    wp = _wpack(g, n, h, w, strides, weights, CONV_FWD)
    _OP.conv2d_fwd_bnstats_abn(x_pre, abn.mean, abn.invstd, abn.weight, abn.bias, list(weights), wp, out, stats,
                               (n, g.cin, h, w), strides, _wshape(g), g.stride, g.pads, g.dils, nt)
    return out, (stats, nt)


def conv_wgrad_abn(g: ConvGeom, dy: torch.Tensor, x_pre: torch.Tensor, abn: OperandBN, n: int, h: int, w: int, dws,
                   accumulate: bool = True) -> None:
    _OP.conv2d_bwd_weight_abn(dy, x_pre, abn.mean, abn.invstd, abn.weight, abn.bias, list(dws), (n, g.cin, h, w),
                              nhwc_strides(n, h, w, g.cin), _wshape(g), g.stride, g.pads, g.dils,
                              EPI_ACCUMULATE if accumulate else 0)


def conv_bnsum_tiles(g: ConvGeom, n: int, h: int, w: int, with_copy: bool = False) -> int:
    d = _desc(g, n, h, w, nhwc_strides(n, h, w, g.cin))[0]
    nt = ctypes.c_int(0)
    check(_lib.lib().adaptseg_conv2d_bnsum_tiles(ctypes.byref(d), 1 if with_copy else 0, ctypes.byref(nt)),
          "conv2d_bnsum_tiles")
    return nt.value


@dataclass
class BnSum:
    x: torch.Tensor
    mean: torch.Tensor
    invstd: torch.Tensor
    weight: torch.Tensor | None
    bias: torch.Tensor | None
    mask: int
    bits: torch.Tensor | None = None


BNSUM_NONE, BNSUM_RELU_X, BNSUM_BITS = 0, 1, 2


def conv_dgrad(g: ConvGeom, dy: torch.Tensor, n: int, h: int, w: int, weights, out=None,
               res=None, aux=None, flags: int = 0, dyb=None, bf16_out: bool = False, bf16_only: bool = False,
               resbits=None, bnsum: BnSum | None = None):
    low = bf16_only or (out is not None and out.dtype == torch.bfloat16)
    dev = (dy if dy is not None else dyb).device
    if out is None:
        out = torch.empty((n, h, w, g.cin), device=dev, dtype=torch.bfloat16 if low else torch.float32)
    if res is not None:
        flags |= EPI_RESIDUAL
    if aux is not None and not flags & EPI_RELU_GRAD:
        assert not low, "conv_dgrad: aux with bf16 gradient storage is not a supported combination"
        flags |= EPI_LEAKY_GRAD
    outb = None if low else _bf16_like(out, bf16_out)
    dx, dxb = (None, out) if low else (out, outb)
    wp = _wpack(g, n, h, w, nhwc_strides(n, h, w, g.cin), weights, CONV_BWD_DATA)
    ret = out if (low or not bf16_out) else (out, outb)
    nt = 0
    if (bnsum is not None and aux is None and g.cin % 4 == 0 and _aligned16(dy, *weights) and
            _aligned16(bnsum.mean, bnsum.invstd, bnsum.weight, bnsum.bias) and
            (bnsum.x is None or bnsum.x.dtype != torch.float32 or _aligned16(bnsum.x))):
        nt = conv_bnsum_tiles(g, n, h, w, with_copy=dyb is not None and _aligned16(dyb))
    if nt == 0:
        _OP.conv2d_bwd_data(dy, dyb, list(weights), wp, res, resbits, aux, dx, dxb, (n, g.cin, h, w), _wshape(g),
                            g.stride, g.pads, g.dils, flags)
        return ret if bnsum is None else (ret, None)
    partial = torch.empty(2 * g.cin * nt, device=dev, dtype=torch.float32)
    b = bnsum
    _OP.conv2d_bwd_data_bnsum(dy, dyb, list(weights), wp, res, resbits, dx, dxb, (n, g.cin, h, w), _wshape(g),
                              g.stride, g.pads, g.dils, flags, b.x, b.mean, b.invstd, b.weight, b.bias, b.bits,
                              int(b.mask), partial, nt)
    return ret, (partial, nt)

# ... 336 lines not shown
```

adaptsegnet_amd/ops.py:

```python
from __future__ import annotations

import ctypes

import torch

from . import _lib
from ._lib import CONV_BWD_DATA, CONV_BWD_WEIGHT, CONV_FWD, MATH_F32X3, ConvDesc, check

LIB = torch.library.Library("adaptseg", "DEF")


def _stream() -> ctypes.c_void_p:
    return ctypes.c_void_p(torch.cuda.current_stream().cuda_stream)


def _p(t):
    return None if t is None else ctypes.c_void_p(t.data_ptr())


def _pf(t, n, what):
    if t is None:
        return None
    if t.dtype != torch.float32 or t.numel() != n:
        raise RuntimeError(f"{what}: expected a float32 tensor of {n} elements, got {t.dtype} {tuple(t.shape)}")
    return ctypes.c_void_p(t.data_ptr())


def _pc(t, n, what):
    if t is None:
        return None
    if t.dtype != torch.bfloat16 or t.numel() not in (n, 3 * n):
        raise RuntimeError(f"{what}: expected a bf16 copy of {n} (or 3 x {n}) elements, got {t.dtype} "
                           f"{tuple(t.shape)}")
    return ctypes.c_void_p(t.data_ptr())


def _pfb(t, n, what):
    if t is None:
        return None, None
    if t.dtype == torch.bfloat16:
        return None, _pc(t, n, what)
    return _pf(t, n, what), None


def _pbits(t, n, what):
    if t is None:
        return None
    if t.dtype != torch.int32 or t.numel() * 32 != n:
        raise RuntimeError(f"{what}: expected an int32 bitmap of {n // 32} words, got {t.dtype} {tuple(t.shape)}")
    return ctypes.c_void_p(t.data_ptr())


def _ptrs(ts):
    return _lib.ptr_array([None if t is None else t.data_ptr() for t in ts])


_WS: dict = {}


def workspace(nbytes: int, device: torch.device):
    if nbytes == 0:
        return None
    key = (device.index, torch.cuda.current_stream(device).cuda_stream)
    buf = _WS.get(key)
    if buf is None or buf.numel() < nbytes:
        cap = max(nbytes, 0 if buf is None else int(buf.numel() * 1.25))
        buf = torch.empty(cap, dtype=torch.uint8, device=device)
        _WS[key] = buf
    return buf


def _ws_args(nbytes: int, device):
    w = workspace(nbytes, device)
    return (ctypes.c_void_p(w.data_ptr()) if w is not None else None), ctypes.c_size_t(nbytes)


_DESC_CACHE: dict = {}
_CONV_MATH = [MATH_F32X3]
OPT_X3H, OPT_G16_WIDE = 1, 2
_OPTS: dict = {}


def get_option(opt: int) -> int:
    if opt not in _OPTS:
        m = ctypes.c_int(0)
        check(_lib.lib().adaptseg_conv_get_option(int(opt), ctypes.byref(m)), "conv_get_option")
        _OPTS[opt] = m.value
    return _OPTS[opt]


def set_option(opt: int, value: int) -> None:
    check(_lib.lib().adaptseg_conv_set_option(int(opt), int(value)), "conv_set_option")
    _OPTS[opt] = int(value)


def conv_desc(n, c, h, w, strides, cout, kh, kw, stride, pads, dils):
    key = (n, c, h, w, strides, cout, kh, kw, stride, pads, dils, _CONV_MATH[0], get_option(OPT_X3H),
           get_option(OPT_G16_WIDE))
    d = _DESC_CACHE.get(key)
    if d is None:
        p, dl = pads[0], dils[0]
        oh = (h + 2 * p - dl * (kh - 1) - 1) // stride + 1
        ow = (w + 2 * p - dl * (kw - 1) - 1) // stride + 1
        desc = ConvDesc()
        desc.n, desc.c, desc.h, desc.w = n, c, h, w
        for i in range(4):
            desc.in_stride[i] = strides[i]
        desc.k, desc.oh, desc.ow = cout, oh, ow
        desc.kh, desc.kw, desc.stride, desc.nseg = kh, kw, stride, len(pads)
        for i in range(len(pads)):
            desc.pad[i] = pads[i]
            desc.dil[i] = dils[i]
        ws = {}
        for op in (CONV_FWD, CONV_BWD_DATA, CONV_BWD_WEIGHT):
            b = ctypes.c_size_t(0)
            check(_lib.lib().adaptseg_conv2d_workspace_size(ctypes.byref(desc), op, ctypes.byref(b)),
                  "conv2d_workspace_size")
            ws[op] = b.value
        d = _DESC_CACHE[key] = (desc, ws, oh, ow)
    return d


def set_math(math: int) -> None:
    check(_lib.lib().adaptseg_conv_set_math(int(math)), "conv_set_math")
    _CONV_MATH[0] = int(math)


def _wdesc(in_shape, in_stride, w_shape, stride, pad, dil):
    co, _ci, kh, kw = w_shape
    n, c, h, w = in_shape
    return conv_desc(n, c, h, w, tuple(in_stride), co, kh, kw, stride, tuple(pad), tuple(dil))


def _prod(shape):
    out = 1
    for v in shape:
        out *= int(v)
    return out


def _nhwc_strides(n, h, w, c):
    return (h * w * c, 1, w * c, c)


def _fake(*args, **kwargs):
    return None


NAMES: list = []


def _op(schema):
    name = schema.split("(", 1)[0]

    def deco(fn):
        NAMES.append(name)
        LIB.define(schema)
        LIB.impl(name, fn, "CUDA")
        torch.library.register_fake(f"adaptseg::{name}", _fake, lib=LIB)
        return fn
    return deco


@_op("conv2d_wpack(Tensor[] weight, Tensor(a!) pack, int[] in_shape, int[] in_stride, int[] w_shape, int stride, "
     "int[] pad, int[] dil, int op) -> ()")
def _conv2d_wpack(weight, pack, in_shape, in_stride, w_shape, stride, pad, dil, op):
    d, _, _, _ = _wdesc(in_shape, in_stride, w_shape, stride, pad, dil)
    check(_lib.lib().adaptseg_conv2d_wpack(ctypes.byref(d), int(op), _ptrs(weight), _p(pack), pack.numel(),
                                           _stream()), "conv2d_wpack")


@_op("conv2d_fwd(Tensor? x, Tensor? xb, Tensor[] weight, Tensor? wpack, Tensor?[] bias, Tensor? res, "
     "Tensor(a!)? out, Tensor(b!)? outb, int[] in_shape, int[] in_stride, int[] w_shape, int stride, int[] pad, "
     "int[] dil, int flags) -> ()")
def _conv2d_fwd(x, xb, weight, wpack, bias, res, out, outb, in_shape, in_stride, w_shape, stride, pad, dil, flags):
    d, ws, oh, ow = _wdesc(in_shape, in_stride, w_shape, stride, pad, dil)
    wp, wsz = _ws_args(ws[CONV_FWD], (out if out is not None else outb).device)
    nx, ny = _prod(in_shape), in_shape[0] * oh * ow * w_shape[0]
    check(_lib.lib().adaptseg_conv2d_fwd_x(
        ctypes.byref(d), _pf(x, nx, "conv2d_fwd x"), _pc(xb, nx, "conv2d_fwd xb"), _ptrs(weight), _p(wpack),
        _ptrs(bias) if len(bias) else None, _pf(res, ny, "conv2d_fwd res"),
        _pf(out, ny, "conv2d_fwd out"), _pc(outb, ny, "conv2d_fwd outb"), flags, wp, wsz, _stream()), "conv2d_fwd")


@_op("conv2d_fwd_bnstats(Tensor? x, Tensor? xb, Tensor[] weight, Tensor? wpack, Tensor(a!)? out, Tensor(c!)? outb, "
     "Tensor(b!) stats, int[] in_shape, int[] in_stride, int[] w_shape, int stride, int[] pad, int[] dil, "
     "int ntiles) -> ()")
def _conv2d_fwd_bnstats(x, xb, weight, wpack, out, outb, stats, in_shape, in_stride, w_shape, stride, pad, dil,
                        ntiles):
    d, ws, oh, ow = _wdesc(in_shape, in_stride, w_shape, stride, pad, dil)
    wp, wsz = _ws_args(ws[CONV_FWD], stats.device)
    nt = ctypes.c_int(0)
    nx, ny = _prod(in_shape), in_shape[0] * oh * ow * w_shape[0]
    check(_lib.lib().adaptseg_conv2d_fwd_bnstats_x(
        ctypes.byref(d), _pf(x, nx, "conv2d_fwd_bnstats x"), _pc(xb, nx, "conv2d_fwd_bnstats xb"), _ptrs(weight),
        _p(wpack), _pf(out, ny, "conv2d_fwd_bnstats out"), _pc(outb, ny, "conv2d_fwd_bnstats outb"), _p(stats),
        ctypes.c_size_t(stats.numel() * 4), ctypes.byref(nt), wp, wsz, _stream()), "conv2d_fwd_bnstats")
    if nt.value != ntiles:
        raise RuntimeError(f"conv2d_fwd_bnstats: planned {ntiles} statistics tiles, the launch produced "
                           f"{nt.value} (unaligned operand?)")


def _abn(mean, invstd, bnw, bnb):
    return _lib.OperandBN(mean.data_ptr(), invstd.data_ptr(), None if bnw is None else bnw.data_ptr(),
                          None if bnb is None else bnb.data_ptr())


_ABN_OK: dict = {}


def operand_bn_ok(in_shape, in_stride, w_shape, stride, pad, dil, op) -> bool:
    key = (tuple(in_shape), tuple(in_stride), tuple(w_shape), stride, tuple(pad), tuple(dil), op, _CONV_MATH[0],
           get_option(OPT_X3H), get_option(OPT_G16_WIDE))
    v = _ABN_OK.get(key)
    if v is None:
        d = _wdesc(in_shape, in_stride, w_shape, stride, pad, dil)[0]
        ok = ctypes.c_int(0)
        check(_lib.lib().adaptseg_conv2d_operand_bn_ok(ctypes.byref(d), int(op), ctypes.byref(ok)), "operand_bn_ok")
        v = _ABN_OK[key] = bool(ok.value)
    return v


@_op("conv2d_fwd_bnstats_abn(Tensor x_pre, Tensor mean, Tensor invstd, Tensor? bnw, Tensor? bnb, Tensor[] weight, "
     "Tensor? wpack, Tensor(a!) out, Tensor(b!) stats, int[] in_shape, int[] in_stride, int[] w_shape, int stride, "
     "int[] pad, int[] dil, int ntiles) -> ()")
def _conv2d_fwd_bnstats_abn(x_pre, mean, invstd, bnw, bnb, weight, wpack, out, stats, in_shape, in_stride, w_shape,
                            stride, pad, dil, ntiles):
    d, ws, oh, ow = _wdesc(in_shape, in_stride, w_shape, stride, pad, dil)
    wp, wsz = _ws_args(ws[CONV_FWD], stats.device)
    nt = ctypes.c_int(0)
    nx, ny = _prod(in_shape), in_shape[0] * oh * ow * w_shape[0]
    a = _abn(mean, invstd, bnw, bnb)
    check(_lib.lib().adaptseg_conv2d_fwd_bnstats_abn(
        ctypes.byref(d), _pf(x_pre, nx, "conv2d_fwd_bnstats_abn x_pre"), ctypes.byref(a), _ptrs(weight), _p(wpack),
        _pf(out, ny, "conv2d_fwd_bnstats_abn out"), _p(stats), ctypes.c_size_t(stats.numel() * 4), ctypes.byref(nt),
        wp, wsz, _stream()), "conv2d_fwd_bnstats_abn")
    if nt.value != ntiles:
        raise RuntimeError(f"conv2d_fwd_bnstats_abn: planned {ntiles} statistics tiles, the launch produced "
                           f"{nt.value} (unaligned operand?)")


@_op("conv2d_bwd_weight_abn(Tensor dy, Tensor x_pre, Tensor mean, Tensor invstd, Tensor? bnw, Tensor? bnb, "
     "Tensor(a!)[] dw, int[] in_shape, int[] in_stride, int[] w_shape, int stride, int[] pad, int[] dil, "
     "int flags) -> ()")
def _conv2d_bwd_weight_abn(dy, x_pre, mean, invstd, bnw, bnb, dw, in_shape, in_stride, w_shape, stride, pad, dil,
                           flags):
    d, ws, oh, ow = _wdesc(in_shape, in_stride, w_shape, stride, pad, dil)
    wp, wsz = _ws_args(ws[CONV_BWD_WEIGHT], dw[0].device)
    nx, ny = _prod(in_shape), in_shape[0] * oh * ow * w_shape[0]
    a = _abn(mean, invstd, bnw, bnb)
    check(_lib.lib().adaptseg_conv2d_bwd_weight_abn(
        ctypes.byref(d), _pf(dy, ny, "conv2d_bwd_weight_abn dy"), _pf(x_pre, nx, "conv2d_bwd_weight_abn x_pre"),
        ctypes.byref(a), _ptrs(dw), flags, wp, wsz, _stream()), "conv2d_bwd_weight_abn")


@_op("bn_fwd_train_tiles_stats(Tensor stats, int ntiles, int rows, int c, Tensor(a!)? running_mean, "
     "Tensor(b!)? running_var, Tensor(d!) mean, Tensor(e!) invstd, float momentum, float eps) -> ()")
def _bn_fwd_train_tiles_stats(stats, ntiles, rows, c, running_mean, running_var, mean, invstd, momentum, eps):
    check(_lib.lib().adaptseg_bn_fwd_train_tiles_stats(
        int(rows), int(c), _p(stats), int(ntiles), _p(running_mean), _p(running_var), float(momentum), float(eps),
        _p(mean), _p(invstd), _stream()), "bn_fwd_train_tiles_stats")


@_op("conv2d_bwd_data(Tensor? dy, Tensor? dyb, Tensor[] weight, Tensor? wpack, Tensor? res, Tensor? resbits, "
     "Tensor? aux, Tensor(a!)? dx, Tensor(b!)? dxb, int[] in_shape, int[] w_shape, int stride, int[] pad, "
     "int[] dil, int flags) -> ()")
def _conv2d_bwd_data(dy, dyb, weight, wpack, res, resbits, aux, dx, dxb, in_shape, w_shape, stride, pad, dil, flags):
    n, c, h, w = in_shape
    d, ws, oh, ow = _wdesc(in_shape, _nhwc_strides(n, h, w, c), w_shape, stride, pad, dil)
    wp, wsz = _ws_args(ws[CONV_BWD_DATA], (dx if dx is not None else dxb).device)
    nx, ny = n * h * w * c, n * oh * ow * w_shape[0]
    check(_lib.lib().adaptseg_conv2d_bwd_data_xg(
        ctypes.byref(d), _pf(dy, ny, "conv2d_bwd_data dy"), _pc(dyb, ny, "conv2d_bwd_data dyb"), _ptrs(weight),
        _p(wpack), *_pfb(res, nx, "conv2d_bwd_data res"), _pbits(resbits, nx, "conv2d_bwd_data resbits"),
        _pf(aux, nx, "conv2d_bwd_data aux"),
        _pf(dx, nx, "conv2d_bwd_data dx"), _pc(dxb, nx, "conv2d_bwd_data dxb"), flags, wp, wsz, _stream()),
        "conv2d_bwd_data")


@_op("conv2d_bwd_data_bnsum(Tensor? dy, Tensor? dyb, Tensor[] weight, Tensor? wpack, Tensor? res, Tensor? resbits, "
     "Tensor(a!)? dx, Tensor(b!)? dxb, int[] in_shape, int[] w_shape, int stride, int[] pad, int[] dil, int flags, "
     "Tensor bnx, Tensor mean, Tensor invstd, Tensor? bnw, Tensor? bnb, Tensor? bits, int mask, Tensor(c!) partial, "
     "int ntiles) -> ()")
def _conv2d_bwd_data_bnsum(dy, dyb, weight, wpack, res, resbits, dx, dxb, in_shape, w_shape, stride, pad, dil, flags,
                           bnx, mean, invstd, bnw, bnb, bits, mask, partial, ntiles):
    n, c, h, w = in_shape
    d, ws, oh, ow = _wdesc(in_shape, _nhwc_strides(n, h, w, c), w_shape, stride, pad, dil)
    wp, wsz = _ws_args(ws[CONV_BWD_DATA], partial.device)
    nx, ny = n * h * w * c, n * oh * ow * w_shape[0]
    if partial.dtype != torch.float32 or partial.numel() != 2 * c * ntiles:
        raise RuntimeError(f"conv2d_bwd_data_bnsum: partial must be float32 [2][{c}][{ntiles}]")
    bs = _lib.BnSumDesc()
    bs.x, bs.x_bf16 = _pfb(bnx, nx, "conv2d_bwd_data_bnsum bnx")
    bs.mean, bs.invstd, bs.weight, bs.bias = _p(mean), _p(invstd), _p(bnw), _p(bnb)
    bs.bits = _pbits(bits, nx, "conv2d_bwd_data_bnsum bits")
    bs.mask = int(mask)
    bs.partial = _p(partial)
    bs.partial_bytes = partial.numel() * 4
    nt = ctypes.c_int(0)
    check(_lib.lib().adaptseg_conv2d_bwd_data_bnsum(
        ctypes.byref(d), _pf(dy, ny, "conv2d_bwd_data_bnsum dy"), _pc(dyb, ny, "conv2d_bwd_data_bnsum dyb"),
        _ptrs(weight), _p(wpack), *_pfb(res, nx, "conv2d_bwd_data_bnsum res"),
        _pbits(resbits, nx, "conv2d_bwd_data_bnsum resbits"), _pf(dx, nx, "conv2d_bwd_data_bnsum dx"),
        _pc(dxb, nx, "conv2d_bwd_data_bnsum dxb"), flags, ctypes.byref(bs), ctypes.byref(nt), wp, wsz, _stream()),
        "conv2d_bwd_data_bnsum")
    if nt.value != ntiles:
        raise RuntimeError(f"conv2d_bwd_data_bnsum: planned {ntiles} BN-sum tiles, the launch produced {nt.value} "
                           f"(unaligned operand?)")


@_op("conv2d_bwd_weight(Tensor? dy, Tensor? dyb, Tensor? x, Tensor? xb, Tensor(a!)[] dw, Tensor(b!)[] db, "
     "int[] in_shape, int[] in_stride, int[] w_shape, int stride, int[] pad, int[] dil, int flags) -> ()")
def _conv2d_bwd_weight(dy, dyb, x, xb, dw, db, in_shape, in_stride, w_shape, stride, pad, dil, flags):
    d, ws, oh, ow = _wdesc(in_shape, in_stride, w_shape, stride, pad, dil)
    if flags & WGRAD_DEFER_SUM:
        nb = ws[CONV_BWD_WEIGHT]
        w = torch.empty(nb, dtype=torch.uint8, device=dw[0].device) if nb else None
        if w is not None:
            _DEFERRED_WS.setdefault(torch.cuda.current_stream(dw[0].device).cuda_stream, []).append(w)
        wp, wsz = (ctypes.c_void_p(w.data_ptr()) if w is not None else None), ctypes.c_size_t(nb)
    else:
        wp, wsz = _ws_args(ws[CONV_BWD_WEIGHT], dw[0].device)
# ... 413 lines not shown
```

include/adaptseg.h:

```cpp
#ifndef ADAPTSEG_H
#define ADAPTSEG_H

#include <stddef.h>
#include <stdint.h>

#ifdef __cplusplus
extern "C" {
#endif

typedef void *adaptseg_stream_t;

enum adaptseg_status {
  ADAPTSEG_OK = 0,
  ADAPTSEG_ERR_ARG = 1,
  ADAPTSEG_ERR_UNSUPPORTED = 2,
  ADAPTSEG_ERR_HIP = 3,
  ADAPTSEG_ERR_WORKSPACE = 4
};

const char *adaptseg_last_error(void);
const char *adaptseg_version(void);

typedef struct adaptseg_conv_desc {
  int n, c, h, w;
  int64_t in_stride[4];
  int k, oh, ow;
  int kh, kw;
  int stride;
  int nseg;
  int pad[4];
  int dil[4];
} adaptseg_conv_desc;

enum adaptseg_conv_op { ADAPTSEG_CONV_FWD = 0, ADAPTSEG_CONV_BWD_DATA = 1, ADAPTSEG_CONV_BWD_WEIGHT = 2 };

enum adaptseg_conv_flags {
  ADAPTSEG_EPI_LEAKY = 1,
  ADAPTSEG_EPI_ACCUMULATE = 2,
  ADAPTSEG_EPI_LEAKY_GRAD = 4,
  ADAPTSEG_EPI_RESIDUAL = 8,
  ADAPTSEG_EPI_RELU = 16,
  ADAPTSEG_EPI_RELU_GRAD = 32,
  ADAPTSEG_WGRAD_DEFER_SUM = 64
};

enum adaptseg_conv_math {
  ADAPTSEG_MATH_F32 = 0,
  ADAPTSEG_MATH_BF16 = 1,
  ADAPTSEG_MATH_BF16_WIDE = 2,
  ADAPTSEG_MATH_F32X3 = 3,
  ADAPTSEG_MATH_F32X3_PRESPLIT = 4
};
int adaptseg_conv_set_math(int math);
int adaptseg_conv_get_math(int *math);
enum adaptseg_conv_option { ADAPTSEG_OPT_X3H = 1, ADAPTSEG_OPT_G16_WIDE = 2 };
int adaptseg_conv_set_option(int option, int value);
int adaptseg_conv_get_option(int option, int *value);

int adaptseg_conv2d_workspace_size(const adaptseg_conv_desc *d, int op, size_t *bytes);
int adaptseg_conv2d_kernel_id(const adaptseg_conv_desc *d, int op, int *kernel_id, int *splits);
int adaptseg_conv2d_kernel_id_x(const adaptseg_conv_desc *d, int op, int with_copies, int *kernel_id, int *splits);

int adaptseg_conv2d_fwd(const adaptseg_conv_desc *d, const float *x, const float *const *w,
                        const float *const *bias, const float *res, float *y, int flags,
                        void *ws, size_t ws_bytes, adaptseg_stream_t stream);

int adaptseg_conv2d_bnstats_size(const adaptseg_conv_desc *d, size_t *bytes);
int adaptseg_conv2d_bnstats_tiles(const adaptseg_conv_desc *d, int *ntiles);
int adaptseg_conv2d_bnstats_tiles_x(const adaptseg_conv_desc *d, int with_copy, int *ntiles);
int adaptseg_conv2d_fwd_bnstats(const adaptseg_conv_desc *d, const float *x, const float *const *w,
                                float *y, float *stats, size_t stats_bytes, int *ntiles, void *ws,
                                size_t ws_bytes, adaptseg_stream_t stream);

int adaptseg_conv2d_copy_operand_only(const adaptseg_conv_desc *d, int op, int *only);

typedef struct {
  const float *mean, *invstd;
  const float *weight, *bias;
} adaptseg_operand_bn;
int adaptseg_conv2d_operand_bn_ok(const adaptseg_conv_desc *d, int op, int *ok);
int adaptseg_conv2d_fwd_bnstats_abn(const adaptseg_conv_desc *d, const float *x_pre, const adaptseg_operand_bn *abn,
                                    const float *const *w, const void *w_pack, float *y, float *stats,
                                    size_t stats_bytes, int *ntiles, void *ws, size_t ws_bytes,
                                    adaptseg_stream_t stream);
int adaptseg_conv2d_bwd_weight_abn(const adaptseg_conv_desc *d, const float *dy, const float *x_pre,
                                   const adaptseg_operand_bn *abn, float *const *dw, int flags, void *ws,
                                   size_t ws_bytes, adaptseg_stream_t stream);
int adaptseg_conv2d_wpack_size(const adaptseg_conv_desc *d, int op, size_t *bytes);
int adaptseg_conv2d_wpack(const adaptseg_conv_desc *d, int op, const float *const *w, void *pack, size_t bytes,
                          adaptseg_stream_t stream);
int adaptseg_conv2d_fwd_x(const adaptseg_conv_desc *d, const float *x, const uint16_t *x_bf16,
                          const float *const *w, const void *w_pack, const float *const *bias, const float *res,
                          float *y, uint16_t *y_bf16, int flags, void *ws, size_t ws_bytes,
                          adaptseg_stream_t stream);
int adaptseg_conv2d_fwd_bnstats_x(const adaptseg_conv_desc *d, const float *x, const uint16_t *x_bf16,
                                  const float *const *w, const void *w_pack, float *y, uint16_t *y_bf16,
                                  float *stats, size_t stats_bytes, int *ntiles, void *ws, size_t ws_bytes,
                                  adaptseg_stream_t stream);
int adaptseg_conv2d_bwd_data_x(const adaptseg_conv_desc *d, const float *dy, const uint16_t *dy_bf16,
                               const float *const *w, const void *w_pack, const float *res, const float *aux,
                               float *dx, uint16_t *dx_bf16, int flags, void *ws, size_t ws_bytes,
                               adaptseg_stream_t stream);
int adaptseg_conv2d_bwd_data_xg(const adaptseg_conv_desc *d, const float *dy, const uint16_t *dy_bf16,
                                const float *const *w, const void *w_pack, const float *res, const uint16_t *res_bf16,
                                const uint32_t *res_bits, const float *aux, float *dx, uint16_t *dx_bf16, int flags,
                                void *ws, size_t ws_bytes, adaptseg_stream_t stream);
typedef struct {
  const float *x;
  const uint16_t *x_bf16;
  const float *mean, *invstd;
  const float *weight, *bias;
  const uint32_t *bits;
  int mask;
  float *partial;
  size_t partial_bytes;
} adaptseg_bnsum_desc;
int adaptseg_conv2d_bnsum_tiles(const adaptseg_conv_desc *d, int with_copy, int *ntiles);
int adaptseg_conv2d_bwd_data_bnsum(const adaptseg_conv_desc *d, const float *dy, const uint16_t *dy_bf16,
                                   const float *const *w, const void *w_pack, const float *res,
                                   const uint16_t *res_bf16, const uint32_t *res_bits, float *dx, uint16_t *dx_bf16,
                                   int flags, const adaptseg_bnsum_desc *bs, int *ntiles, void *ws, size_t ws_bytes,
                                   adaptseg_stream_t stream);
int adaptseg_conv2d_bwd_weight_x(const adaptseg_conv_desc *d, const float *dy, const uint16_t *dy_bf16,
                                 const float *x, const uint16_t *x_bf16, float *const *dw,
                                 float *const *db, int flags, void *ws, size_t ws_bytes,
                                 adaptseg_stream_t stream);

int adaptseg_conv2d_bwd_data(const adaptseg_conv_desc *d, const float *dy, const float *const *w,
                             const float *res, const float *aux, float *dx, int flags, void *ws,
                             size_t ws_bytes, adaptseg_stream_t stream);

int adaptseg_conv2d_bwd_weight(const adaptseg_conv_desc *d, const float *dy, const float *x,
                               float *const *dw, float *const *db, int flags, void *ws,
                               size_t ws_bytes, adaptseg_stream_t stream);

int adaptseg_splitk_flush(adaptseg_stream_t stream);
int adaptseg_splitk_pending(adaptseg_stream_t stream, int *count);

int adaptseg_bn_workspace_size(int64_t rows, int c, size_t *bytes);

int adaptseg_bn_fwd_train(int64_t rows, int c, const float *x, const float *weight,
                          const float *bias, float *running_mean, float *running_var,
                          float momentum, float eps, float *save_mean, float *save_invstd,
                          const float *res, float *y, int relu, void *ws, size_t ws_bytes,
                          adaptseg_stream_t stream);

int adaptseg_bn_fwd_train_tiles(int64_t rows, int c, const float *stats, int ntiles, const float *x,
                                const float *weight, const float *bias, float *running_mean,
                                float *running_var, float momentum, float eps, float *save_mean,
                                float *save_invstd, const float *res, float *y, int relu,
                                adaptseg_stream_t stream);

int adaptseg_bn_fwd_train_x(int64_t rows, int c, const float *x, const uint16_t *x_bf16, const float *weight,
                            const float *bias, float *running_mean, float *running_var, float momentum, float eps,
                            float *save_mean, float *save_invstd, const float *res, const uint16_t *res_bf16,
                            float *y, uint16_t *y_bf16, int relu, void *ws, size_t ws_bytes,
                            adaptseg_stream_t stream);
int adaptseg_bn_fwd_train_tiles_stats(int64_t rows, int c, const float *stats, int ntiles, float *running_mean,
                                      float *running_var, float momentum, float eps, float *save_mean,
                                      float *save_invstd, adaptseg_stream_t stream);
int adaptseg_bn_fwd_train_tiles_x(int64_t rows, int c, const float *stats, int ntiles, const float *x,
                                  const uint16_t *x_bf16, const float *weight, const float *bias,
                                  float *running_mean, float *running_var, float momentum, float eps,
                                  float *save_mean, float *save_invstd, const float *res, const uint16_t *res_bf16,
                                  float *y, uint16_t *y_bf16, int relu, adaptseg_stream_t stream);
int adaptseg_bn_fwd_infer_x(int64_t rows, int c, const float *x, const uint16_t *x_bf16, const float *weight,
                            const float *bias, const float *running_mean, const float *running_var, float eps,
                            const float *res, const uint16_t *res_bf16, float *y, uint16_t *y_bf16, int relu,
                            adaptseg_stream_t stream);
int adaptseg_bn_fwd_train_xm(int64_t rows, int c, const float *x, const uint16_t *x_bf16, const float *weight,
                             const float *bias, float *running_mean, float *running_var, float momentum, float eps,
                             float *save_mean, float *save_invstd, const float *res, const uint16_t *res_bf16,
                             float *y, uint16_t *y_bf16, uint32_t *relu_bits, int relu, void *ws, size_t ws_bytes,
                             adaptseg_stream_t stream);
int adaptseg_bn_fwd_train_tiles_xm(int64_t rows, int c, const float *stats, int ntiles, const float *x,
                                   const uint16_t *x_bf16, const float *weight, const float *bias,
                                   float *running_mean, float *running_var, float momentum, float eps,
                                   float *save_mean, float *save_invstd, const float *res, const uint16_t *res_bf16,
                                   float *y, uint16_t *y_bf16, uint32_t *relu_bits, int relu, adaptseg_stream_t stream);
int adaptseg_bn_fwd_infer_xm(int64_t rows, int c, const float *x, const uint16_t *x_bf16, const float *weight,
                             const float *bias, const float *running_mean, const float *running_var, float eps,
                             const float *res, const uint16_t *res_bf16, float *y, uint16_t *y_bf16,
                             uint32_t *relu_bits, int relu, adaptseg_stream_t stream);

int adaptseg_bn_fwd_infer(int64_t rows, int c, const float *x, const float *weight,
                          const float *bias, const float *running_mean, const float *running_var,
                          float eps, const float *res, float *y, int relu,
                          adaptseg_stream_t stream);

int adaptseg_bn_bwd(int64_t rows, int c, const float *dy, const float *y, const float *x,
                    const float *weight, const float *bias, const float *save_mean,
                    const float *save_invstd, float *dx, float *dres, int relu, int train,
                    void *ws, size_t ws_bytes, adaptseg_stream_t stream);

int adaptseg_bn_bwd_x(int64_t rows, int c, const float *dy, const float *y, const uint16_t *y_bf16, const float *x,
                      const uint16_t *x_bf16, const float *weight, const float *bias, const float *save_mean,
                      const float *save_invstd, float *dx, uint16_t *dx_bf16, float *dres, int relu, int train,
                      void *ws, size_t ws_bytes, adaptseg_stream_t stream);

int adaptseg_bn_bwd_xg(int64_t rows, int c, const float *dy, const uint16_t *dy_bf16, const uint32_t *dy_bits,
                       const float *y, const uint16_t *y_bf16, const float *x, const uint16_t *x_bf16,
                       const float *weight, const float *bias, const float *save_mean, const float *save_invstd,
                       float *dx, uint16_t *dx_bf16, float *dres, uint16_t *dres_bf16, int relu, int train, void *ws,
                       size_t ws_bytes, adaptseg_stream_t stream);

int adaptseg_bn_bwd_sums(int64_t rows, int c, const float *dy, const uint16_t *dy_bf16, const uint32_t *dy_bits,
                         const float *y, const uint16_t *y_bf16, const float *x, const uint16_t *x_bf16,
                         const float *weight, const float *bias, const float *save_mean, const float *save_invstd,
                         float *dx, uint16_t *dx_bf16, float *dres, uint16_t *dres_bf16, int relu,
                         const float *partial, int ntiles, void *ws, size_t ws_bytes, adaptseg_stream_t stream);

int adaptseg_bn_bwd_affine(int64_t rows, int c, const float *dy, const float *y, const float *x,
                           const float *weight, const float *bias, const float *save_mean,
                           const float *save_invstd, float *dx, float *dres, int act, float *dweight,
                           float *dbias, void *ws, size_t ws_bytes, adaptseg_stream_t stream);

int adaptseg_upsample_argmax(int n, int c, int h, int w, int oh, int ow, const float *x,
                             uint8_t *out, adaptseg_stream_t stream);
#define ADAPTSEG_FUSE_MAX_MAPS 8
#define ADAPTSEG_FUSE_PROB 0
#define ADAPTSEG_FUSE_LOGIT 1
typedef struct adaptseg_fuse_desc {
  int n, c, oh, ow, nmaps, mode;
  int h[ADAPTSEG_FUSE_MAX_MAPS], w[ADAPTSEG_FUSE_MAX_MAPS], mirror[ADAPTSEG_FUSE_MAX_MAPS];
  const float *x[ADAPTSEG_FUSE_MAX_MAPS];
} adaptseg_fuse_desc;
int adaptseg_fuse_argmax(const adaptseg_fuse_desc *d, uint8_t *out, float *conf, adaptseg_stream_t stream);
int adaptseg_confusion_hist(int64_t npix, const uint8_t *gt, const int32_t *lut,
                            const uint8_t *pred, int ncls, int64_t *hist, adaptseg_stream_t stream);

int adaptseg_conf_hist(int64_t npix, const uint8_t *pred, const float *conf, int ncls, int nbins,
                       int64_t *hist, adaptseg_stream_t stream);
int adaptseg_pseudo_thresholds(const int64_t *hist, int ncls, int nbins, double portion, float cap,
                               float *thr, adaptseg_stream_t stream);
int adaptseg_pseudo_label(int64_t npix, const uint8_t *pred, const float *conf, const float *thr,
                          int ncls, int ignore_label, int64_t *labels, int64_t *kept,
                          adaptseg_stream_t stream);

int adaptseg_preprocess_workspace_size(int n, int in_h, int in_w, int out_h, int out_w, size_t *bytes);
int adaptseg_gta5_preprocess(int n, int in_h, int in_w, int out_h, int out_w, const uint8_t *rgb, float mean_b,
                             float mean_g, float mean_r, float *image, const uint8_t *label_ids, const int32_t *lut,
                             int64_t *labels, void *ws, size_t ws_bytes, adaptseg_stream_t stream);
int adaptseg_preprocess_augment_workspace_size(int n, int in_h, int in_w, int out_h, int out_w,
// ... 90 lines not shown
```

Before: 30.45 images/s.

## Batch per-step weight repacking into one launch per math family

Records which weight packs were used in the previous training step and, at the start of the next weight_pack_scope, rebuilds all of them with a single batched kernel per family (x3 and bf16). The batch uses a device-side item table with prefix offsets and a binary search. This replaces many small per-layer wpack launches and their host dispatch overhead. It adds table construction, validity checks and a pinned-memory upload, and packs are rebuilt eagerly even if a later call would have hit the cache.

Result: no change. 30.55 images/s (median of 5 runs) (+0.3%).

```diff
diff --git a/adaptsegnet_amd/_lib.py b/adaptsegnet_amd/_lib.py
--- a/adaptsegnet_amd/_lib.py
+++ b/adaptsegnet_amd/_lib.py
@@ -48,6 +48,20 @@
         ("bits", ctypes.c_void_p), ("mask", ctypes.c_int),
         ("partial", ctypes.c_void_p), ("partial_bytes", ctypes.c_size_t),
     ]
+
+
+WPACK_BATCH_MAX = 4096
+WPACK_TABLE_MAGIC = 0x4B505741
+
+
+class WpackItem(ctypes.Structure):
+    _fields_ = [("desc", ConvDesc), ("op", ctypes.c_int), ("w", ctypes.c_void_p * 4),
+                ("pack", ctypes.c_void_p), ("bytes", ctypes.c_size_t)]
+
+
+class WpackTableHeader(ctypes.Structure):
+    _fields_ = [(f, ctypes.c_uint32) for f in ("magic", "n", "n_x3", "n_bf16", "units_x3", "units_bf16",
+                                               "first_off", "items_off")]
 
 
 FUSE_MAX_MAPS = 8
@@ -89,6 +103,9 @@
     "adaptseg_conv2d_bwd_weight": [_DESC, _P, _P, _PP, _PP, _I, _P, _SZ, _P],
     "adaptseg_conv2d_wpack_size": [_DESC, _I, ctypes.POINTER(_SZ)],
     "adaptseg_conv2d_wpack": [_DESC, _I, _PP, _P, _SZ, _P],
+    "adaptseg_conv2d_wpack_batch_size": [_I, ctypes.POINTER(_SZ)],
+    "adaptseg_conv2d_wpack_batch_table": [ctypes.POINTER(WpackItem), _I, _P, _SZ],
+    "adaptseg_conv2d_wpack_batch": [_P, _P, _SZ, _P],
     "adaptseg_conv2d_fwd_x": [_DESC, _P, _P, _PP, _P, _PP, _P, _P, _P, _I, _P, _SZ, _P],
     "adaptseg_conv2d_fwd_bnstats_x": [_DESC, _P, _P, _PP, _P, _P, _P, _P, _SZ, ctypes.POINTER(ctypes.c_int), _P,
                                       _SZ, _P],
@@ -206,6 +223,8 @@
         except OSError as e:
             raise AdaptSegLibraryError(f"failed to load {LIB_PATH}: {e}") from e
         for name, argtypes in _SIGS.items():
+            if name in _BATCH_SYMS and os.environ.get("ADAPTSEG_LIBRARY") and not hasattr(L, name):
+                continue
             fn = getattr(L, name)
             fn.argtypes = argtypes
             fn.restype = _RESTYPES.get(name, ctypes.c_int)
@@ -213,6 +232,14 @@
         return L
 
 
+_BATCH_SYMS = ("adaptseg_conv2d_wpack_batch_size", "adaptseg_conv2d_wpack_batch_table",
+               "adaptseg_conv2d_wpack_batch")
+
+
+def has_wpack_batch() -> bool:
+    return all(hasattr(lib(), s) for s in _BATCH_SYMS)
+
+
 def check(status: int, what: str) -> None:
     if status != ADAPTSEG_OK:
         msg = lib().adaptseg_last_error().decode(errors="replace")
diff --git a/adaptsegnet_amd/csrc/conv_igemm.hip b/adaptsegnet_amd/csrc/conv_igemm.hip
--- a/adaptsegnet_amd/csrc/conv_igemm.hip
+++ b/adaptsegnet_amd/csrc/conv_igemm.hip
@@ -951,9 +951,8 @@
   return ADAPTSEG_OK;
 }
 
-int adaptseg_conv2d_wpack(const adaptseg_conv_desc *d, int op, const float *const *w, void *pack, size_t bytes,
-                          adaptseg_stream_t stream) {
-  Plan pl;
+static int wpack_plan(const adaptseg_conv_desc *d, int op, const float *const *w, const void *pack, size_t bytes,
+                      Plan &pl) {
   int st = make_plan(d, op, pl);
   if (st) return st;
   AS_CHECK_ARG(w && pack, "conv2d_wpack: null pointer");
@@ -966,9 +965,110 @@
     AS_CHECK_ARG(aligned16(w[s]), "conv2d_wpack: weight %d must be 16-byte aligned", s);
     pl.p.wt[s] = w[s];
   }
+  return ADAPTSEG_OK;
+}
+
+int adaptseg_conv2d_wpack(const adaptseg_conv_desc *d, int op, const float *const *w, void *pack, size_t bytes,
+                          adaptseg_stream_t stream) {
+  Plan pl;
+  int st = wpack_plan(d, op, w, pack, bytes, pl);
+  if (st) return st;
   const hipError_t e = is_x3(pl.family) ? prep_x3_wpack(pl, pack, as_stream(stream)) : prep_bf16_wpack(pl, pack, as_stream(stream));
   if (e != hipSuccess) {
     set_error("conv2d_wpack: %s", hipGetErrorString(e));
+    return ADAPTSEG_ERR_HIP;
+  }
+  return ADAPTSEG_OK;
+}
+
+static size_t wpack_items_off(int n) { return (sizeof(adaptseg_wpack_table_header) + 4 * ((size_t)n + 2) + 63) / 64 * 64; }
+static size_t wpack_table_bytes(int n) { return wpack_items_off(n) + (size_t)n * sizeof(WpackItem); }
+static_assert(sizeof(WpackItem) % 16 == 0 && sizeof(adaptseg_wpack_table_header) == 32, "wpack table layout");
+
+int adaptseg_conv2d_wpack_batch_size(int n, size_t *table_bytes) {
+  AS_CHECK_ARG(table_bytes, "conv2d_wpack_batch_size: null");
+  AS_CHECK_ARG(n > 0 && n <= ADAPTSEG_WPACK_BATCH_MAX, "conv2d_wpack_batch_size: n = %d not in [1, %d]", n,
+               ADAPTSEG_WPACK_BATCH_MAX);
+  *table_bytes = wpack_table_bytes(n);
+  return ADAPTSEG_OK;
+}
+
+int adaptseg_conv2d_wpack_batch_table(const adaptseg_wpack_item *items, int n, void *host_table, size_t table_bytes) {
+  AS_CHECK_ARG(items && host_table, "conv2d_wpack_batch_table: null pointer");
+  AS_CHECK_ARG(n > 0 && n <= ADAPTSEG_WPACK_BATCH_MAX, "conv2d_wpack_batch_table: n = %d not in [1, %d]", n,
+               ADAPTSEG_WPACK_BATCH_MAX);
+  AS_CHECK_ARG(table_bytes >= wpack_table_bytes(n), "conv2d_wpack_batch_table: %zu bytes < %zu", table_bytes,
+               wpack_table_bytes(n));
+  AS_CHECK_ARG((reinterpret_cast<uintptr_t>(host_table) & 15) == 0,
+               "conv2d_wpack_batch_table: table must be 16-byte aligned");
+  std::vector<WpackItem> its[2];
+  std::vector<uint32_t> units[2];
+  uint64_t sum[2] = {0, 0};
+  for (int i = 0; i < n; ++i) {
+    const adaptseg_wpack_item &a = items[i];
+    Plan pl;
+    const int st = wpack_plan(&a.desc, a.op, a.w, a.pack, a.bytes, pl);
+    if (st) return st;
+    const int f = is_x3(pl.family) ? 0 : 1;
+    WpackItem it;
+    std::memset(&it, 0, sizeof(it));
+    const uint32_t u = f == 0 ? x3_wpack_item(pl, a.pack, it) : bf16_wpack_item(pl, a.pack, it);
+    sum[f] += u;
+    AS_CHECK_ARG(u > 0 && sum[f] < (uint64_t)1 << 31, "conv2d_wpack_batch_table: item %d: too many work units", i);
+    its[f].push_back(it);
+    units[f].push_back(u);
+  }
+  char *base = reinterpret_cast<char *>(host_table);
+  std::memset(base, 0, wpack_table_bytes(n));
+  adaptseg_wpack_table_header h;
+  h.magic = ADAPTSEG_WPACK_TABLE_MAGIC;
+  h.n = (uint32_t)n;
+  h.n_x3 = (uint32_t)its[0].size();
+  h.n_bf16 = (uint32_t)its[1].size();
+  h.units_x3 = (uint32_t)sum[0];
+  h.units_bf16 = (uint32_t)sum[1];
+  h.first_off = (uint32_t)sizeof(h);
+  h.items_off = (uint32_t)wpack_items_off(n);
+  std::memcpy(base, &h, sizeof(h));
+  uint32_t *first = reinterpret_cast<uint32_t *>(base + h.first_off);
+  WpackItem *out = reinterpret_cast<WpackItem *>(base + h.items_off);
+  for (int f = 0; f < 2; ++f) {
+    uint32_t acc = 0;
+    *first++ = 0;
+    for (size_t i = 0; i < its[f].size(); ++i) {
+      acc += units[f][i];
+      *first++ = acc;
+      std::memcpy(out++, &its[f][i], sizeof(WpackItem));
+    }
+  }
+  return ADAPTSEG_OK;
+}
+
+int adaptseg_conv2d_wpack_batch(const void *host_table, const void *table, size_t table_bytes,
+                                adaptseg_stream_t stream) {
+  AS_CHECK_ARG(host_table && table, "conv2d_wpack_batch: null pointer");
+  AS_CHECK_ARG(table_bytes >= sizeof(adaptseg_wpack_table_header), "conv2d_wpack_batch: %zu bytes hold no table",
+               table_bytes);
+  adaptseg_wpack_table_header h;
+  std::memcpy(&h, host_table, sizeof(h));
+  AS_CHECK_ARG(h.magic == ADAPTSEG_WPACK_TABLE_MAGIC && h.n > 0 && h.n <= ADAPTSEG_WPACK_BATCH_MAX &&
+                   h.n_x3 + h.n_bf16 == h.n && h.first_off == sizeof(h) && h.items_off == wpack_items_off((int)h.n),
+               "conv2d_wpack_batch: host_table is no table of adaptseg_conv2d_wpack_batch_table");
+  AS_CHECK_ARG(table_bytes >= wpack_table_bytes((int)h.n), "conv2d_wpack_batch: %zu bytes < %zu", table_bytes,
+               wpack_table_bytes((int)h.n));
+  AS_CHECK_ARG((reinterpret_cast<uintptr_t>(table) & 15) == 0, "conv2d_wpack_batch: table must be 16-byte aligned");
+  const uint32_t *hf = reinterpret_cast<const uint32_t *>(reinterpret_cast<const char *>(host_table) + h.first_off);
+  AS_CHECK_ARG(hf[0] == 0 && hf[h.n_x3] == h.units_x3 && hf[h.n_x3 + 1] == 0 && hf[h.n + 1] == h.units_bf16,
+               "conv2d_wpack_batch: host_table's prefixes do not match its header");
+  const char *base = reinterpret_cast<const char *>(table);
+  const uint32_t *first = reinterpret_cast<const uint32_t *>(base + h.first_off);
+  const WpackItem *its = reinterpret_cast<const WpackItem *>(base + h.items_off);
+  hipError_t e = hipSuccess;
+  if (h.n_x3) e = x3_wpack_batch(its, first, (int)h.n_x3, h.units_x3, as_stream(stream));
+  if (e == hipSuccess && h.n_bf16)
+    e = bf16_wpack_batch(its + h.n_x3, first + h.n_x3 + 1, (int)h.n_bf16, h.units_bf16, as_stream(stream));
+  if (e != hipSuccess) {
+    set_error("conv2d_wpack_batch: %s", hipGetErrorString(e));
     return ADAPTSEG_ERR_HIP;
   }
   return ADAPTSEG_OK;
diff --git a/adaptsegnet_amd/csrc/conv_kernels.hpp b/adaptsegnet_amd/csrc/conv_kernels.hpp
--- a/adaptsegnet_amd/csrc/conv_kernels.hpp
+++ b/adaptsegnet_amd/csrc/conv_kernels.hpp
@@ -55,6 +55,29 @@
 };
 constexpr int kAbnMaxC = 512;
 
+enum {
+  WPACK_X3_FWD = 0, WPACK_X3_DGRAD = 1,
+  WPACK_BF16_FWD_V = 2, WPACK_BF16_FWD = 3,
+  WPACK_BF16_DGRAD_V = 4, WPACK_BF16_DGRAD = 5,
+};
+struct WpackItem {
+  ConvParams p;
+  char *pack;
+  int kind;
+  int ktot;
+  uint32_t cpr, total;
+  uint32_t gx, gy;
+};
+__device__ __forceinline__ int wpack_find_item(const uint32_t *__restrict__ first, int n, uint32_t u) {
+  int lo = 0, hi = n;
+  while (hi - lo > 1) {
+    const int mid = (lo + hi) >> 1;
+    if (first[mid] <= u) lo = mid;
+    else hi = mid;
+  }
+  return lo;
+}
+
 __device__ __forceinline__ float epi_prev(const ConvParams &p, size_t idx) {
   return p.out ? p.out[idx] : (float)p.outb[idx];
 }
@@ -1612,6 +1635,10 @@
 hipError_t prep_x3(const Plan &pl, void *wpack, hipStream_t s);
 hipError_t prep_x3_wpack(const Plan &pl, void *pack, hipStream_t s);
 hipError_t launch_x3(const Plan &pl, void *wpack, hipStream_t s);
+uint32_t x3_wpack_item(const Plan &pl, void *pack, WpackItem &it);
+uint32_t bf16_wpack_item(const Plan &pl, void *pack, WpackItem &it);
+hipError_t x3_wpack_batch(const WpackItem *items, const uint32_t *first, int n, uint32_t units, hipStream_t s);
+hipError_t bf16_wpack_batch(const WpackItem *items, const uint32_t *first, int n, uint32_t units, hipStream_t s);
 hipError_t launch_dgrad(const Plan &pl, hipStream_t s);
 hipError_t launch_wgrad(const Plan &pl, hipStream_t s);
 
diff --git a/adaptsegnet_amd/csrc/conv_launch_bf16.hip b/adaptsegnet_amd/csrc/conv_launch_bf16.hip
--- a/adaptsegnet_amd/csrc/conv_launch_bf16.hip
+++ b/adaptsegnet_amd/csrc/conv_launch_bf16.hip
@@ -3,19 +3,21 @@
 
 namespace adaptseg {
 
+__device__ __forceinline__ void wpack_fwd_body(const ConvParams &p, __bf16 *out, int ktot, int64_t i) {
+  const int co = (int)(i / ktot), kk = (int)(i - (int64_t)co * ktot);
+  const int seg = kk / p.kseg, tk = kk - seg * p.kseg;
+  out[i] = (__bf16)seg_ptr(p, seg)[(size_t)co * p.kseg + tk];
+}
 __global__ void conv_wpack_fwd_kernel(const ConvParams p, __bf16 *out) {
   const int ktot = p.nseg * p.kseg;
   const int64_t n = (int64_t)p.k * ktot;
-  for (int64_t i = (int64_t)blockIdx.x * blockDim.x + threadIdx.x; i < n; i += (int64_t)gridDim.x * blockDim.x) {
-    const int co = (int)(i / ktot), kk = (int)(i - (int64_t)co * ktot);
-    const int seg = kk / p.kseg, tk = kk - seg * p.kseg;
-    out[i] = (__bf16)seg_ptr(p, seg)[(size_t)co * p.kseg + tk];
-  }
-}
-
-__global__ void __launch_bounds__(256) conv_wpack_dgrad_kernel(const ConvParams p, __bf16 *out) {
-  __shared__ float tile[64][65];
-  const int ci0 = blockIdx.x * 64, co0 = blockIdx.y * 64, tap = blockIdx.z;
+  for (int64_t i = (int64_t)blockIdx.x * blockDim.x + threadIdx.x; i < n; i += (int64_t)gridDim.x * blockDim.x)
+    wpack_fwd_body(p, out, ktot, i);
+}
+
+__device__ __forceinline__ void wpack_dgrad_body(const ConvParams &p, __bf16 *out, float (*tile)[65], int bx, int by,
+                                                 int tap) {
+  const int ci0 = bx * 64, co0 = by * 64;
   const int seg = tap / p.taps_per_seg, t = tap - seg * p.taps_per_seg;
   const float *w = seg_ptr(p, seg);
   const int tx = threadIdx.x & 63, ty = threadIdx.x >> 6;
@@ -30,23 +32,29 @@
     if (ci < p.c && co < p.k) out[(size_t)ci * ktot + (size_t)tap * p.k + co] = (__bf16)tile[tx][r];
   }
 }
-
+__global__ void __launch_bounds__(256) conv_wpack_dgrad_kernel(const ConvParams p, __bf16 *out) {
+  __shared__ float tile[64][65];
+  wpack_dgrad_body(p, out, tile, blockIdx.x, blockIdx.y, blockIdx.z);
+}
+
+__device__ __forceinline__ void wpack_fwd_v_body(const ConvParams &p, uint4 *__restrict__ out, uint32_t cpr,
+                                                 uint32_t i) {
+  const uint32_t co = i / cpr, k0 = (i - co * cpr) * 8;
+  int seg = 0;
+  uint32_t tk = k0;
+  while (tk >= (uint32_t)p.kseg) { tk -= p.kseg; ++seg; }
+  const float *src = seg_ptr(p, seg) + (size_t)co * p.kseg + tk;
+  const uint2 lo = cvt4_bf16(ld4(src)), hi = cvt4_bf16(ld4(src + 4));
+  out[i] = make_uint4(lo.x, lo.y, hi.x, hi.y);
+}
 __global__ void __launch_bounds__(256) conv_wpack_fwd_v_kernel(const ConvParams p, uint4 *__restrict__ out,
                                                                uint32_t cpr, uint32_t total) {
-  for (uint32_t i = blockIdx.x * 256u + threadIdx.x; i < total; i += gridDim.x * 256u) {
-    const uint32_t co = i / cpr, k0 = (i - co * cpr) * 8;
-    int seg = 0;
-    uint32_t tk = k0;
-    while (tk >= (uint32_t)p.kseg) { tk -= p.kseg; ++seg; }
-    const float *src = seg_ptr(p, seg) + (size_t)co * p.kseg + tk;
-    const uint2 lo = cvt4_bf16(ld4(src)), hi = cvt4_bf16(ld4(src + 4));
-    out[i] = make_uint4(lo.x, lo.y, hi.x, hi.y);
-  }
-}
-
-__global__ void __launch_bounds__(256) conv_wpack_dgrad_v_kernel(const ConvParams p, __bf16 *out) {
-  __shared__ float tile[64][65];
-  const int ci0 = blockIdx.x * 64, co0 = blockIdx.y * 64, tap = blockIdx.z;
+  for (uint32_t i = blockIdx.x * 256u + threadIdx.x; i < total; i += gridDim.x * 256u) wpack_fwd_v_body(p, out, cpr, i);
+}
+
+__device__ __forceinline__ void wpack_dgrad_v_body(const ConvParams &p, __bf16 *out, float (*tile)[65], int bx,
+                                                   int by, int tap) {
+  const int ci0 = bx * 64, co0 = by * 64;
   const int seg = tap / p.taps_per_seg, t = tap - seg * p.taps_per_seg;
   const float *w = seg_ptr(p, seg);
   const int f = threadIdx.x & 15, r0 = threadIdx.x >> 4;
@@ -68,6 +76,31 @@
     const uint2 lo = cvt4_bf16(make_float4(col[0], col[65], col[130], col[195]));
     const uint2 hi = cvt4_bf16(make_float4(col[260], col[325], col[390], col[455]));
     *reinterpret_cast<uint4 *>(out + (size_t)ci * ktot + (size_t)tap * p.k + co) = make_uint4(lo.x, lo.y, hi.x, hi.y);
+  }
+}
+__global__ void __launch_bounds__(256) conv_wpack_dgrad_v_kernel(const ConvParams p, __bf16 *out) {
+  __shared__ float tile[64][65];
+  wpack_dgrad_v_body(p, out, tile, blockIdx.x, blockIdx.y, blockIdx.z);
+}
+
+__global__ void __launch_bounds__(256) conv_wpack_bf16_batch_kernel(const WpackItem *__restrict__ items,
+                                                                    const uint32_t *__restrict__ first, int n) {
+  __shared__ float tile[64][65];
+  const int i = wpack_find_item(first, n, blockIdx.x);
+  const WpackItem &it = items[i];
+  const uint32_t u = blockIdx.x - first[i];
+  __bf16 *out = reinterpret_cast<__bf16 *>(it.pack);
+  if (it.kind == WPACK_BF16_FWD_V) {
+    const uint32_t j = u * 256u + threadIdx.x;
+    if (j < it.total) wpack_fwd_v_body(it.p, reinterpret_cast<uint4 *>(out), it.cpr, j);
+  } else if (it.kind == WPACK_BF16_FWD) {
+    const int ktot = it.p.nseg * it.p.kseg;
+    const int64_t j = (int64_t)u * 256 + threadIdx.x;
+    if (j < (int64_t)it.p.k * ktot) wpack_fwd_body(it.p, out, ktot, j);
+  } else {
+    const uint32_t z = u / (it.gx * it.gy), r = u - z * (it.gx * it.gy), y = r / it.gx, x = r - y * it.gx;
+    if (it.kind == WPACK_BF16_DGRAD_V) wpack_dgrad_v_body(it.p, out, tile, (int)x, (int)y, (int)z);
+    else wpack_dgrad_body(it.p, out, tile, (int)x, (int)y, (int)z);
   }
 }
 
@@ -109,14 +142,25 @@
   return 0;
 }
 
-hipError_t prep_bf16_wpack(const Plan &pl, void *pack, hipStream_t s) {
-  const ConvParams &p = pl.p;
-  __bf16 *wb = reinterpret_cast<__bf16 *>(pack);
+static int bf16_wpack_kind(const Plan &pl) {
+  const ConvParams &p = pl.p;
   bool wal = true;
   for (int g = 0; g < p.nseg; ++g) wal = wal && (reinterpret_cast<uintptr_t>(p.wt[g]) & 15) == 0;
   if (pl.mode == MODE_FWD) {
     const int64_t n = (int64_t)p.k * p.nseg * p.kseg;
-    if (wal && p.kseg % 8 == 0 && n / 8 < (int64_t)1 << 31) {
+    return wal && p.kseg % 8 == 0 && n / 8 < (int64_t)1 << 31 ? WPACK_BF16_FWD_V : WPACK_BF16_FWD;
+  }
+  if (pl.mode == MODE_DGRAD) return wal && p.c % 4 == 0 && p.k % 8 == 0 ? WPACK_BF16_DGRAD_V : WPACK_BF16_DGRAD;
+  return -1;
+}
+
+hipError_t prep_bf16_wpack(const Plan &pl, void *pack, hipStream_t s) {
+  const ConvParams &p = pl.p;
+  __bf16 *wb = reinterpret_cast<__bf16 *>(pack);
+  const int kind = bf16_wpack_kind(pl);
+  if (pl.mode == MODE_FWD) {
+    const int64_t n = (int64_t)p.k * p.nseg * p.kseg;
+    if (kind == WPACK_BF16_FWD_V) {
       const uint32_t total = (uint32_t)(n / 8);
       conv_wpack_fwd_v_kernel<<<(unsigned)std::min<int64_t>(ceil_div(total, 256), 4096), 256, 0, s>>>(
           p, reinterpret_cast<uint4 *>(wb), (uint32_t)(p.nseg * p.kseg / 8), total);
@@ -125,9 +169,39 @@
     }
   } else if (pl.mode == MODE_DGRAD) {
     dim3 g((unsigned)ceil_div(p.c, 64), (unsigned)ceil_div(p.k, 64), (unsigned)p.ntaps);
-    if (wal && p.c % 4 == 0 && p.k % 8 == 0) conv_wpack_dgrad_v_kernel<<<g, 256, 0, s>>>(p, wb);
+    if (kind == WPACK_BF16_DGRAD_V) conv_wpack_dgrad_v_kernel<<<g, 256, 0, s>>>(p, wb);
     else conv_wpack_dgrad_kernel<<<g, 256, 0, s>>>(p, wb);
   }
+  return hipGetLastError();
+}
+
+uint32_t bf16_wpack_item(const Plan &pl, void *pack, WpackItem &it) {
+  const ConvParams &p = pl.p;
+  it.p = p;
+  it.pack = reinterpret_cast<char *>(pack);
+  it.kind = bf16_wpack_kind(pl);
+  it.ktot = 0;
+  it.cpr = it.total = it.gx = it.gy = 0;
+  int64_t units = 0;
+  if (pl.mode == MODE_FWD) {
+    const int64_t n = (int64_t)p.k * p.nseg * p.kseg;
+    if (it.kind == WPACK_BF16_FWD_V) {
+      it.cpr = (uint32_t)(p.nseg * p.kseg / 8);
+      it.total = (uint32_t)(n / 8);
+      units = ceil_div(n / 8, 256);
+    } else {
+      units = ceil_div(n, 256);
+    }
+  } else if (pl.mode == MODE_DGRAD) {
+    it.gx = (uint32_t)ceil_div(p.c, 64);
+    it.gy = (uint32_t)ceil_div(p.k, 64);
+    units = (int64_t)it.gx * it.gy * p.ntaps;
+  }
+  return units < (int64_t)1 << 31 ? (uint32_t)units : 0;
+}
+
+hipError_t bf16_wpack_batch(const WpackItem *items, const uint32_t *first, int n, uint32_t units, hipStream_t s) {
+  conv_wpack_bf16_batch_kernel<<<units, 256, 0, s>>>(items, first, n);
   return hipGetLastError();
 }
 
diff --git a/adaptsegnet_amd/csrc/conv_launch_x3.hip b/adaptsegnet_amd/csrc/conv_launch_x3.hip
--- a/adaptsegnet_amd/csrc/conv_launch_x3.hip
+++ b/adaptsegnet_amd/csrc/conv_launch_x3.hip
@@ -51,6 +51,22 @@
   const dim3 pg((unsigned)(rows_pad / x3_bn(pl.mode)), (unsigned)(ktot / kX3BK));
   if (pl.mode == MODE_FWD) conv_wpack_x3v_kernel<MODE_FWD><<<pg, 256, 0, s>>>(p, (char *)pack, ktot);
   else if (pl.mode == MODE_DGRAD) conv_wpack_x3v_kernel<MODE_DGRAD><<<pg, 256, 0, s>>>(p, (char *)pack, ktot);
+  return hipGetLastError();
+}
+
+uint32_t x3_wpack_item(const Plan &pl, void *pack, WpackItem &it) {
+  int rows_pad, ktot;
+  x3_pack_dims(pl, rows_pad, ktot);
+  it.p = pl.p;
+  it.pack = reinterpret_cast<char *>(pack);
+  it.kind = pl.mode == MODE_FWD ? WPACK_X3_FWD : WPACK_X3_DGRAD;
+  it.ktot = ktot;
+  it.cpr = it.total = it.gx = it.gy = 0;
+  return (uint32_t)(rows_pad / x3_bn(pl.mode)) * (uint32_t)(ktot / kX3BK);
+}
+
+hipError_t x3_wpack_batch(const WpackItem *items, const uint32_t *first, int n, uint32_t units, hipStream_t s) {
+  conv_wpack_x3v_batch_kernel<<<units, 256, 0, s>>>(items, first, n);
   return hipGetLastError();
 }
 
diff --git a/adaptsegnet_amd/csrc/conv_x3.hpp b/adaptsegnet_amd/csrc/conv_x3.hpp
--- a/adaptsegnet_amd/csrc/conv_x3.hpp
+++ b/adaptsegnet_amd/csrc/conv_x3.hpp
@@ -380,11 +380,11 @@
 }
 
 template <int MODE>
-__global__ void __launch_bounds__(256) conv_wpack_x3v_kernel(const ConvParams p, char *out, int ktot) {
+__device__ __forceinline__ void wpack_x3v_body(const ConvParams &p, char *out, int ktot, int bx, int ks) {
   constexpr int TR = x3_bn(MODE), IMGB = TR * kX3BK * 2;
   const int r = threadIdx.x >> 1, ch = threadIdx.x & 1;
-  const int n = blockIdx.x * TR + r;
-  const int ks = blockIdx.y, k0 = ks * kX3BK + 8 * ch;
+  const int n = bx * TR + r;
+  const int k0 = ks * kX3BK + 8 * ch;
   float v[8];
   if constexpr (MODE == MODE_FWD) {
     if (n < p.k) {
@@ -410,10 +410,25 @@
   split3_2(v[4], v[5], h.z, m.z, l.z);
   split3_2(v[6], v[7], h.w, m.w, l.w);
   const int nkt = ktot / kX3BK;
-  char *dst = out + ((size_t)blockIdx.x * nkt + ks) * 3 * IMGB + kc16_off(r, ch);
+  char *dst = out + ((size_t)bx * nkt + ks) * 3 * IMGB + kc16_off(r, ch);
   *reinterpret_cast<uint4 *>(dst) = h;
   *reinterpret_cast<uint4 *>(dst + IMGB) = m;
   *reinterpret_cast<uint4 *>(dst + 2 * IMGB) = l;
 }
 
-}
+template <int MODE>
+__global__ void __launch_bounds__(256) conv_wpack_x3v_kernel(const ConvParams p, char *out, int ktot) {
+  wpack_x3v_body<MODE>(p, out, ktot, blockIdx.x, blockIdx.y);
+}
+
+__global__ void __launch_bounds__(256) conv_wpack_x3v_batch_kernel(const WpackItem *__restrict__ items,
+                                                                   const uint32_t *__restrict__ first, int n) {
+  const int i = wpack_find_item(first, n, blockIdx.x);
+  const WpackItem &it = items[i];
+  const uint32_t u = blockIdx.x - first[i], nkt = (uint32_t)(it.ktot / kX3BK);
+  const int bx = (int)(u / nkt), ks = (int)(u - (uint32_t)bx * nkt);
+  if (it.kind == WPACK_X3_FWD) wpack_x3v_body<MODE_FWD>(it.p, it.pack, it.ktot, bx, ks);
+  else wpack_x3v_body<MODE_DGRAD>(it.p, it.pack, it.ktot, bx, ks);
+}
+
+}
diff --git a/adaptsegnet_amd/kernels.py b/adaptsegnet_amd/kernels.py
--- a/adaptsegnet_amd/kernels.py
+++ b/adaptsegnet_amd/kernels.py
@@ -18,7 +18,7 @@
     "bn_fwd_train_tiles", "bn_fwd_infer", "bn_bwd",
     "maxpool_fwd", "maxpool_bwd", "upsample_fwd", "upsample_bwd", "softmax_fwd", "softmax_bwd",
     "ce_fwd", "ce_bwd", "adv_fwd", "adv_bwd", "sgd_step", "adam_step", "zero_", "to_nhwc",
-    "axpy", "add_i64", "weight_pack_scope", "pack_builds", "pack_count", "clear_weight_packs", "EPI_ACCUMULATE", "EPI_LEAKY", "EPI_LEAKY_GRAD", "EPI_RELU", "EPI_RELU_GRAD", "EPI_RESIDUAL",
+    "axpy", "add_i64", "weight_pack_scope", "pack_builds", "pack_batch_launches", "set_pack_batching", "pack_count", "clear_weight_packs", "EPI_ACCUMULATE", "EPI_LEAKY", "EPI_LEAKY_GRAD", "EPI_RELU", "EPI_RELU_GRAD", "EPI_RESIDUAL",
 ]
 
 
@@ -89,6 +89,23 @@
     return _ops.conv_desc(n, g.cin, h, w, strides, g.cout, g.kh, g.kw, g.stride, g.pads, g.dils)
 
 
+@dataclass
+class _PackUse:
+    weights: tuple
+    shape: tuple
+    strides: tuple
+    size: int
+    opts: tuple
+
+
+@dataclass
+class _PackTable:
+    host: torch.Tensor
+    dev: torch.Tensor
+    packs: tuple
+    families: int
+
+
 class _PackCache:
 
     def __init__(self):
@@ -98,6 +115,38 @@
         self.finalizers = {}
         self.sizes = {}
         self.builds = 0
+        self.used = {}
+        self.step = {}
+        self.table = None
+        self.batch = True
+        self.batch_launches = 0
+        self.table_uploads = 0
+
+    def note_use(self, weights, key, shape, strides, size):
+        k = (id(weights[0]), key)
+        if k not in self.used:
+            self.used[k] = _PackUse(tuple(weakref.ref(t) for t in weights), tuple(shape), tuple(strides), size,
+                                    (_ops.get_option(_ops.OPT_X3H), _ops.get_option(_ops.OPT_G16_WIDE)))
+
+    def end_step(self):
+        if [(k, u.shape, u.strides) for k, u in self.used.items()] != \
+                [(k, u.shape, u.strides) for k, u in self.step.items()]:
+            self.table = None
+        self.step, self.used = self.used, {}
+
+    def still_valid(self):
+        out = []
+        opts = (_ops.get_option(_ops.OPT_X3H), _ops.get_option(_ops.OPT_G16_WIDE)) if self.step else None
+        for (wid, key), u in self.step.items():
+            ws = [r() for r in u.weights]
+            e = self.entries.get(wid, {}).get(key)
+            if (e is None or any(t is None for t in ws) or id(ws[0]) != wid or
+                    tuple(t.data_ptr() for t in ws) != key[0] or not _aligned16(*ws) or
+                    key[3] != _ops._CONV_MATH[0] or u.opts != opts or e[0].numel() < u.size):
+                self.step, self.table = {}, None
+                return None
+            out.append(e)
+        return out or None
 
     def _drop(self, wid):
         self.entries.pop(wid, None)
@@ -121,15 +170,70 @@
 def weight_pack_scope():
     _PACKS.depth += 1
     try:
+        if _PACKS.depth == 1:
+            _build_recorded_packs()
         yield
     finally:
         _PACKS.depth -= 1
         if _PACKS.depth == 0:
             _PACKS.epoch += 1
+            _PACKS.end_step()
+
+
+def _build_recorded_packs():
+    c = _PACKS
+    if not c.batch or not c.step or not _lib.has_wpack_batch():
+        return
+    entries = c.still_valid()
+    if entries is None or len(entries) > _lib.WPACK_BATCH_MAX:
+        return
+    if any(e[0].device != entries[0][0].device for e in entries):
+        return
+    packs = tuple(e[0].data_ptr() for e in entries)
+    if c.table is None or c.table.packs != packs:
+        c.table = _make_pack_table(c, entries, packs)
+    t = c.table
+    _OP.conv2d_wpack_batch(t.host.data_ptr(), t.dev, [e[0] for e in entries])
+    for e in entries:
+        e[1] = c.epoch
+    c.builds += len(entries)
+    c.batch_launches += t.families
+
+
+def _make_pack_table(c, entries, packs):
+    n = len(entries)
+    items = (_lib.WpackItem * n)()
+    for it, ((wid, key), u), e in zip(items, c.step.items(), entries):
+        _ptrs, g, op, _math = key
+        it.desc = _desc(g, u.shape[0], u.shape[1], u.shape[2], u.strides)[0]
+        it.op = op
+        for s, p in enumerate(key[0]):
+            it.w[s] = p
+        it.pack = e[0].data_ptr()
+        it.bytes = e[0].numel()
+    b = ctypes.c_size_t(0)
+    check(_lib.lib().adaptseg_conv2d_wpack_batch_size(n, ctypes.byref(b)), "conv2d_wpack_batch_size")
+    dev = entries[0][0].device
+    host = torch.zeros(b.value, dtype=torch.uint8, pin_memory=dev.type == "cuda")
+    check(_lib.lib().adaptseg_conv2d_wpack_batch_table(items, n, ctypes.c_void_p(host.data_ptr()), b.value),
+          "conv2d_wpack_batch_table")
+    table = torch.empty(b.value, dtype=torch.uint8, device=dev)
+    table.copy_(host, non_blocking=True)
+    c.table_uploads += 1
+    h = _lib.WpackTableHeader.from_address(host.data_ptr())
+    return _PackTable(host, table, packs, int(h.n_x3 > 0) + int(h.n_bf16 > 0))
 
 
 def pack_builds() -> int:
     return _PACKS.builds
+
+
+def pack_batch_launches() -> int:
+    return _PACKS.batch_launches
+
+
+def set_pack_batching(on: bool) -> None:
+    _PACKS.batch = bool(on)
 
 
 def pack_count() -> int:
@@ -165,6 +269,7 @@
                          g.dils, op)
         e[1] = _PACKS.epoch
         _PACKS.builds += 1
+    _PACKS.note_use(weights, key, (n, h, w), strides, size)
     return e[0]
 
 
diff --git a/adaptsegnet_amd/ops.py b/adaptsegnet_amd/ops.py
--- a/adaptsegnet_amd/ops.py
+++ b/adaptsegnet_amd/ops.py
@@ -168,6 +168,12 @@
     d, _, _, _ = _wdesc(in_shape, in_stride, w_shape, stride, pad, dil)
     check(_lib.lib().adaptseg_conv2d_wpack(ctypes.byref(d), int(op), _ptrs(weight), _p(pack), pack.numel(),
                                            _stream()), "conv2d_wpack")
+
+
+@_op("conv2d_wpack_batch(int host_table, Tensor table, Tensor(a!)[] packs) -> ()")
+def _conv2d_wpack_batch(host_table, table, packs):
+    check(_lib.lib().adaptseg_conv2d_wpack_batch(ctypes.c_void_p(host_table), _p(table), table.numel(), _stream()),
+          "conv2d_wpack_batch")
 
 
 @_op("conv2d_fwd(Tensor? x, Tensor? xb, Tensor[] weight, Tensor? wpack, Tensor?[] bias, Tensor? res, "
diff --git a/include/adaptseg.h b/include/adaptseg.h
--- a/include/adaptseg.h
+++ b/include/adaptseg.h
@@ -89,6 +89,22 @@
 int adaptseg_conv2d_wpack_size(const adaptseg_conv_desc *d, int op, size_t *bytes);
 int adaptseg_conv2d_wpack(const adaptseg_conv_desc *d, int op, const float *const *w, void *pack, size_t bytes,
                           adaptseg_stream_t stream);
+#define ADAPTSEG_WPACK_BATCH_MAX 4096
+#define ADAPTSEG_WPACK_TABLE_MAGIC 0x4b505741u
+typedef struct adaptseg_wpack_item {
+  adaptseg_conv_desc desc;
+  int op;
+  const float *w[4];
+  void *pack;
+  size_t bytes;
+} adaptseg_wpack_item;
+typedef struct adaptseg_wpack_table_header {
+  uint32_t magic, n, n_x3, n_bf16, units_x3, units_bf16, first_off, items_off;
+} adaptseg_wpack_table_header;
+int adaptseg_conv2d_wpack_batch_size(int n, size_t *table_bytes);
+int adaptseg_conv2d_wpack_batch_table(const adaptseg_wpack_item *items, int n, void *host_table, size_t table_bytes);
+int adaptseg_conv2d_wpack_batch(const void *host_table, const void *table, size_t table_bytes,
+                                adaptseg_stream_t stream);
 int adaptseg_conv2d_fwd_x(const adaptseg_conv_desc *d, const float *x, const uint16_t *x_bf16,
                           const float *const *w, const void *w_pack, const float *const *bias, const float *res,
                           float *y, uint16_t *y_bf16, int flags, void *ws, size_t ws_bytes,
```
